# fumiama/Retrieval-based-Voice-Conversion-WebUI

Measured on AMD Instinct MI355X. Metric: real-time factor (audio-sec/wall-sec), 48 kHz v2, 10 s clips, retrieval + NSF-HiFi-GAN decode, higher is better.
Workload: dtype fp16 MFMA operands + fp16 inter-stage streams (ResBlock outputs, ups output of stages 1-3), fp32 accumulate / in-block residual; fp32 MFMA prefilter + fp64 verified IVF distances; 1 GPU; BASELINE configs[1]: v2/48k, 1 x 10 s clip(s) per GPU, T=1198 frames, 599 queries/clip, IVF 10000x768 nlist=256 nprobe=1 k=8 index_rate=0.75; hipgraph=True, index_blob_bytes=32376576, launcher=single process

## Files before the change

### retrieval-based-voice-conversion-webui_amd/csrc/nsf.hip

```cpp
#include <algorithm>
#include <atomic>
#include <cmath>
#include <functional>
#include <memory>
#include <string>
#include <unordered_map>

#include "common.hpp"
#include "nsf_kernels.hpp"
#include "conv_pack.hpp"
#include "rb_stream.hpp"

namespace rvcmi {

struct Geom {
    int MI, NJ, WCO, TT;
};
static Geom conv_geom(int cout) {
    Geom g;
    g.NJ = 4;
    if (cout >= 256) { g.MI = 2; g.WCO = 4; }
    else if (cout >= 128) { g.MI = 2; g.WCO = 2; }
    else if (cout >= 64) { g.MI = 2; g.WCO = 1; }
    else { g.MI = 1; g.WCO = 1; }
// ... 1008 lines not shown
    a2.in = hbuf;
    a2.in_mode = IN_OP_RAW;
    a2.out_mode = OUT_F32;
    a2.out = dst;
    a2.res = src;
    a2.res_bstride = L * C;
    for (ConvArgs* a : {&a1, &a2}) {
        a->in_bstride = L * C;
        a->Lin = (int)L;
        a->Lq = (int)L;
        a->lens = f.lens;
        a->lmul_in = a->lmul_q = lm;
        a->out_bstride = L * C;
        a->out_C = C;
    }
}

static void rb_f32_chain(const Fwd& f, const Stage& s, long L, int lm, const float** src) {
    rvcmi_nsf* h = f.h;
    char nm[48];
    snprintf(nm, sizeof(nm), "rb_c%d", s.cout);
    for (size_t j = 0; j < s.rb.size(); ++j)
        for (size_t m = 0; m < s.rb[j].size(); ++m) {
            float* dst = ydst(h, j, m);
            ConvArgs a1, a2;
            rb_pair_args(f, L, s.cout, lm, src[j], h->H.p, dst, a1, a2);
            run_conv(h, s.rb[j][m].first, a1, f.B, nm, f.st);
            run_conv(h, s.rb[j][m].second, a2, f.B, nm, f.st);
            src[j] = dst;
        }
}

static void rb_split(const Fwd& f, const Stage& s, long L, int lm, const float** src) {
    rvcmi_nsf* h = f.h;
    char nm[48];
    snprintf(nm, sizeof(nm), "rb_split_c%d", s.cout);
    for (size_t m = 0; m < max_levels(s); ++m) {
        const ConvLayer* L1[3];
        const ConvLayer* L2[3];
        ConvArgs a1[3], a2[3];
        int nj = 0;
        for (size_t j = 0; j < s.rb.size(); ++j) {
            if (m >= s.rb[j].size()) continue;
            float* dst = ydst(h, j, m);
            void* hbuf = (char*)h->H.p + (size_t)nj * (h->H.bytes / 3);
            rb_pair_args(f, L, s.cout, lm, src[j], hbuf, dst, a1[nj], a2[nj]);
            L1[nj] = &s.rb[j][m].first;
            L2[nj] = &s.rb[j][m].second;
            src[j] = dst;
            ++nj;
        }
        run_conv_jobs(h, L1, a1, nj, f.B, nm, f.st);
        run_conv_jobs(h, L2, a2, nj, f.B, nm, f.st);
    }
}

static void rb_stream(const Fwd& f, const Stage& s, const StagePlan& p, long L, int lm, const float** src) {
    rvcmi_nsf* h = f.h;
    const int C = s.cout, nk = (int)s.rb.size();
    RbStreamDesc sd[3];
    double flops = 0, bytes = 0;
    stream_jobs(f, s, L, lm, p.x0_half, p.stage_half, sd, flops, bytes);
    char nm[48];
    snprintf(nm, sizeof(nm), "rb_stream_c%d", C);
    h->prof.launch(nm, flops, bytes, f.st, [&] {
        rb_stream_launch(f.op, C, 3, sd, nk, (int)L, f.B, L * C, rb_stream_mode(h) == 1, f.st, h->opt);
    });
    HIP_CHECK(hipGetLastError());
    for (int j = 0; j < nk; ++j) src[j] = h->Ya[j].as<float>();
}

static void rb_full(const Fwd& f, const Stage& s, const StagePlan& p, long L, int lm, const float** src) {
    rvcmi_nsf* h = f.h;
    const int C = s.cout, nk = (int)s.rb.size(), B = f.B;
    char nm[48];
    snprintf(nm, sizeof(nm), "rb_full_c%d", C);
    RbFullArgs ra;
    memset(&ra, 0, sizeof(ra));
    ra.L = (int)L;
    ra.lens = f.lens;
    ra.lmul = lm;
    ra.bstride = L * C;
    ra.dbg = dbg_flags(h);
    ra.yh = p.stage_half ? 1 : 0;
    ra.xh = p.x0_half ? 1 : 0;
    ra.pad_tap = h->opt.geti("RBF_PAD_TAP", 0) != 0 ? 1 : 0;
    const int R = p.tall32 ? RBF32T_ROWS : (p.small64 ? RBF64S_ROWS : rbf_rows(C));
    int order[RVCMI_MAX_RB];
    rb_order(s, order);
    int max_tiles = 0;
    double flops = 0, bytes = 0;
    for (int oj = 0; oj < nk; ++oj) {
        const int j = order[oj];
        RbFullJob& J = ra.job[oj];
        J.src = h->X0.as<float>();
        J.dst = h->Ya[j].as<float>();
        J.nd = (int)s.rb[j].size();
        fill_rb_job(J, s.rb[j], 0, J.nd, L, B, C, flops, bytes);
        for (int m = 0; m < J.nd; ++m)
            if (J.dil[m] * (J.k - 1) / 2 + J.dil[m] > RBF_G) RVCMI_FAIL(RVCMI_ERR_INVALID, "dilation too large for the fused resblock");
        J.HL = rbf_halo(s.rb[j]);
        J.tvalid = R - 2 * J.HL;
        if (J.tvalid < R / 4) RVCMI_FAIL(RVCMI_ERR_INVALID, "resblock halo too large for the fused kernel");
        J.ntiles = (int)((L + J.tvalid - 1) / J.tvalid);
        max_tiles = std::max(max_tiles, J.ntiles);
        bytes += (double)B * L * C * ((p.stage_half ? 2 : 4) + (p.x0_half ? 2 : 4));
        src[j] = J.dst;
    }
    const size_t nblk = (size_t)max_tiles * nk * B;
    if (ra.dbg & 32) ra.ts = stamp_buffer(h, nblk * 8 * 16, f.st);
    h->prof.launch(nm, flops, bytes, f.st, [&] {
        if (f.op == RVCMI_OPERAND_BF16) launch_rbf_t<__bf16>(C, ra, max_tiles, nk, B, f.st, p.small64, p.tall32);
        else launch_rbf_t<_Float16>(C, ra, max_tiles, nk, B, f.st, p.small64, p.tall32);
    });
    HIP_CHECK(hipGetLastError());
    if (ra.dbg & 32) {
        const int nwv = p.tall32 ? RBF32T_NWV : (p.small64 ? RBF64S_NWV : (C == 64 ? RbFullGeom<64>::NWV : RBF32_NWV));
        print_stamps(h, nm, ra, nk, max_tiles, nwv, 16, nblk, f.st);
    }
}

static void rb_pair(const Fwd& f, const Stage& s, long L, int lm, const float** src) {
    rvcmi_nsf* h = f.h;
    const int op = f.op, C = s.cout, nk = (int)s.rb.size(), B = f.B;
    const int mode = rb_stream_mode(h);
    char nm[48], nms[48];
    snprintf(nm, sizeof(nm), "rb_pair_c%d", C);
    snprintf(nms, sizeof(nms), "rb_stream1_c%d", C);
    int order[RVCMI_MAX_RB];
    rb_order(s, order);
    constexpr int NWp = 8;
    for (size_t m = 0; m < max_levels(s); ++m) {
        RbPairArgs ra;
        memset(&ra, 0, sizeof(ra));
        ra.lens = f.lens;
        ra.lmul = lm;
        ra.L = (int)L;
        ra.bstride = L * C;
        ra.dbg = dbg_flags(h);
        RbStreamDesc sd[RVCMI_MAX_RB];
        float* dsts[RVCMI_MAX_RB] = {nullptr};
        int nj = 0, max_tiles = 0, max_rows = 0;
        double flops = 0, bytes = 0;
        for (int oj = 0; oj < nk; ++oj) {
            const int j = order[oj];
            if (m >= s.rb[j].size()) continue;
            RbStreamDesc& d = sd[nj];
            memset(&d, 0, sizeof(d));
            d.src = src[j];
            d.dst = dsts[j] = ydst(h, j, m);
            d.lens = f.lens;
            d.lmul = lm;
            fill_rb_job(d, s.rb[j], (int)m, 1, L, B, C, flops, bytes);
            bytes += (double)B * L * C * 8;
            RbJob& J = ra.job[nj++];
            J.src = d.src; J.dst = d.dst; J.w1 = d.w1[0]; J.w2 = d.w2[0]; J.b1 = d.b1[0]; J.b2 = d.b2[0];
            J.ct1 = d.ct1; J.ct2 = d.ct2; J.k = d.k; J.k_p = d.k_p; J.dil = d.dil[0];
            J.tt2 = rb_rows(C) - (J.k - 1);
            J.ntiles = (int)((L + J.tt2 - 1) / J.tt2);
            max_tiles = std::max(max_tiles, J.ntiles);
            max_rows = std::max(max_rows, rb_rows(C) + (J.k_p - 1) * J.dil);
        }
        const size_t nblk = (size_t)max_tiles * nj * B;
        if (ra.dbg & 32) ra.ts = stamp_buffer(h, nblk * NWp * 8, f.st);
        bool streamed = false;
        if (mode != 0 && rb_stream_supported(op, C, 1) && rb_stream_launch(op, C, 1, sd, nj, (int)L, B, L * C, mode == 1, f.st, h->opt, true))
            h->prof.launch(nms, flops, bytes, f.st, [&] { streamed = rb_stream_launch(op, C, 1, sd, nj, (int)L, B, L * C, mode == 1, f.st, h->opt); });
        if (!streamed) h->prof.launch(nm, flops, bytes, f.st, [&] { launch_rb_pair(op, C, ra, max_tiles, nj, B, max_rows, f.st); });
        if ((ra.dbg & 32) && m == 0) print_stamps(h, nm, ra, nj, max_tiles, NWp, 8, nblk, f.st);
        for (int j = 0; j < nk; ++j)
            if (dsts[j]) src[j] = dsts[j];
    }
    HIP_CHECK(hipGetLastError());
}

static void conv_post(const Fwd& f, const Act& x, float* out) {
    rvcmi_nsf* h = f.h;
    const int B = f.B, C = x.C, L = (int)x.L;
    hipStream_t st = f.st;
    const int dbg = h->opt.geti("POST_DBG", 0);
    h->prof.launch("conv_post", 2.0 * 7 * C * (double)x.L * B, (double)B * x.L * (C * h->cfg.n_resblock_kernels * (x.half ? 2 : 4) + 4), st, [&] {
        if (x.half && x.y[1] && x.y[2] && x.div == 3.f && (C == 32 || C == 16) && h->opt.geti("POST_DMA", 1) != 0) {
            const int ntiles = (L + POSTD_TT - 1) / POSTD_TT;
            const dim3 grid((unsigned)std::min(ntiles, std::max(1, num_cus() * 3 / B)), B);
            const _Float16* y0 = (const _Float16*)x.y[0];
            const _Float16* y1 = (const _Float16*)x.y[1];
            const _Float16* y2 = (const _Float16*)x.y[2];
            if (C == 32)
                hipLaunchKernelGGL(k_post_dma<32>, grid, dim3(POSTD_TT), post_dma_smem<32>(), st, y0, y1, y2, h->post_w.as<float>(), out, L, f.lens, x.lm, dbg);
            else
                hipLaunchKernelGGL(k_post_dma<16>, grid, dim3(POSTD_TT), post_dma_smem<16>(), st, y0, y1, y2, h->post_w.as<float>(), out, L, f.lens, x.lm, dbg);
            return;
        }
        const size_t smem = (size_t)(7 * C + (POST_TT + 6) * (C + 4)) * 4;
        hipLaunchKernelGGL(k_post, dim3((unsigned)((L + POST_TT - 1) / POST_TT), B), dim3(256), smem, st, x.y[0], x.y[1], x.y[2],
                           h->post_w.as<float>(), out, L, C, x.div, x.half ? 1 : 0, f.lens, x.lm, dbg);
    });
    HIP_CHECK(hipGetLastError());
}

static void tap_x0(const Fwd& f, const StagePlan& p, long L, int C) {
    rvcmi_nsf* h = f.h;
    if (!p.x0_half) return copy_tap_cl(h, h->X0.as<float>(), f.B, (int)L, C, f.tr, f.st);
    const size_t n = (size_t)f.B * L * C;
    hipLaunchKernelGGL(k_h2f, dim3((unsigned)((n + 255) / 256)), dim3(256), 0, f.st, (const _Float16*)h->X0.p, h->Ya[0].as<float>(), n);
    copy_tap_cl(h, h->Ya[0].as<float>(), f.B, (int)L, C, f.tr, f.st);
}

static void tap_stage(const Fwd& f, const Act& x) {
    rvcmi_nsf* h = f.h;
    const size_t n = (size_t)f.B * x.L * x.C;
    const dim3 grid((unsigned)((n + 255) / 256));
    if (x.half)
        hipLaunchKernelGGL(k_sum3h, grid, dim3(256), 0, f.st, (const _Float16*)x.y[0], (const _Float16*)x.y[1], (const _Float16*)x.y[2],
                           h->X0.as<float>(), n);
    else
        hipLaunchKernelGGL(k_sum3, grid, dim3(256), 0, f.st, x.y[0], x.y[1], x.y[2], h->X0.as<float>(), n);
    copy_tap_cl(h, h->X0.as<float>(), f.B, (int)x.L, x.C, f.tr, f.st);
}

static void nsf_forward(rvcmi_nsf* h, int B, int T, const int* lens, const float* x, const float* f0, const float* g,
                        const float* noise, int n_res, float* out, hipStream_t st, TapRequest* tr) {
    if (!h || !x || (!out && !tr)) RVCMI_FAIL(RVCMI_ERR_INVALID, "null argument");
    if (lens && n_res >= 0) RVCMI_FAIL(RVCMI_ERR_INVALID, "lengths and n_res (the realtime interpolation) cannot be combined");
    const rvcmi_nsf_config& c = h->cfg;
    if (c.use_f0 && !f0) RVCMI_FAIL(RVCMI_ERR_INVALID, "f0 is required for an NSF (use_f0) generator");
    if (B < 1 || T < 1) RVCMI_FAIL(RVCMI_ERR_INVALID, "B and T must be positive");
    const int Te = n_res >= 0 ? n_res : T;
    if (Te < 1) RVCMI_FAIL(RVCMI_ERR_INVALID, "n_res must be positive");
    if (B > h->max_B || T > h->max_T || Te > h->max_T)
        RVCMI_FAIL(RVCMI_ERR_NOMEM, "shape B=%d T=%d n_res=%d exceeds handle limits (max_B=%d max_T=%d)", B, T, n_res,
                   h->max_B, h->max_T);
    HIP_CHECK(hipSetDevice(h->device));
    Fwd f{h, c.operand, B, Te, lens, nullptr, st, tr};
    if (c.use_f0 && excitation(f, T, f0, noise)) return;
    Act a = conv_pre(f, x, T, g);
    if (f.want("pre")) return copy_tap_cl(h, a.y[0], B, Te, h->C0, tr, st);
    char nm[48];
    for (int i = 0; i < c.n_ups; ++i) {
        const Stage& s = h->stages[i];
        const long L = a.L * s.u;
        const int lm = a.lm * s.u, C = s.cout;
        const StagePlan p = plan_stage(f, s, L, lm);
        if (f.op == RVCMI_OPERAND_F32) ups_f32(f, s, a, L, lm);
        else ups_mfma(f, s, a, p, L, lm);
        snprintf(nm, sizeof(nm), "up%d", i);
        if (f.want(nm)) return tap_x0(f, p, L, C);
        const float* src[RVCMI_MAX_RB];
        for (auto& v : src) v = h->X0.as<float>();
        switch (p.path) {
            case RbPath::F32_CHAIN: rb_f32_chain(f, s, L, lm, src); break;
            case RbPath::SPLIT: rb_split(f, s, L, lm, src); break;
            case RbPath::STREAM: rb_stream(f, s, p, L, lm, src); break;
            case RbPath::FULL: rb_full(f, s, p, L, lm, src); break;
            case RbPath::PAIR: rb_pair(f, s, L, lm, src); break;
        }
        const int nk = (int)s.rb.size();
        a = Act{{src[0], nk > 1 ? src[1] : nullptr, nk > 2 ? src[2] : nullptr}, p.stage_half, false, (float)nk, L, C, lm};
        snprintf(nm, sizeof(nm), "stage%d", i);
        if (f.want(nm)) return tap_stage(f, a);
    }
    if (tr) RVCMI_FAIL(RVCMI_ERR_INVALID, "unknown tap '%s'", tr->what);
    conv_post(f, a, out);
}

}

extern "C" {

int rvcmi_nsf_create(const rvcmi_nsf_config* cfg, const rvcmi_tensor* weights, int n_weights, int device, int max_B,
                     int max_T, rvcmi_nsf** out) {
    return guarded([&] { nsf_create(cfg, weights, n_weights, device, max_B, max_T, out); });
}
int rvcmi_nsf_destroy(rvcmi_nsf* h) {
    return guarded([&] { delete h; });
}
int rvcmi_nsf_forward(rvcmi_nsf* h, int B, int T, const int* lengths, const float* x, const float* f0, const float* g,
                      const float* noise, int n_res, float* out, void* stream) {
    return guarded([&] { nsf_forward(h, B, T, lengths, x, f0, g, noise, n_res, out, (hipStream_t)stream, nullptr); });
}
int rvcmi_nsf_upp(const rvcmi_nsf* h) { return h ? h->upp : RVCMI_ERR_INVALID; }
size_t rvcmi_nsf_workspace_bytes(const rvcmi_nsf* h) { return h ? h->ws_bytes : 0; }

int rvcmi_nsf_debug_forward(rvcmi_nsf* h, int B, int T, const float* x, const float* f0, const float* g,
                            const float* noise, int n_res, const char* what, float* out_host, size_t capacity_floats,
                            int64_t shape_out[3], void* stream) {
    return guarded([&] {
        if (!what || !out_host || !shape_out) RVCMI_FAIL(RVCMI_ERR_INVALID, "null argument");
        TapRequest tr;
        tr.what = what;
        tr.out_host = out_host;
        tr.capacity = capacity_floats;
        tr.shape = shape_out;
        nsf_forward(h, B, T, nullptr, x, f0, g, noise, n_res, nullptr, (hipStream_t)stream, &tr);
        if (!tr.done) RVCMI_FAIL(RVCMI_ERR_INVALID, "tap '%s' was not produced", what);
    });
}

int rvcmi_nsf_set_option(rvcmi_nsf* h, const char* key, double value) {
    return guarded([&] {
        if (!h || !key) RVCMI_FAIL(RVCMI_ERR_INVALID, "null argument");
        if ((!strcmp(key, "RBF_PAD_TAP") || !strcmp(key, "RBF32_TALL")) && value == value && value != 0.0 && value != 1.0)
            RVCMI_FAIL(RVCMI_ERR_INVALID, "option '%s' takes 0 or 1", key);
        if (!h->opt.set(key, value)) RVCMI_FAIL(RVCMI_ERR_INVALID, "unknown option '%s' for this handle", key);
    });
}
int rvcmi_nsf_profile_enable(rvcmi_nsf* h, int enable) {
    return guarded([&] {
        if (!h) RVCMI_FAIL(RVCMI_ERR_INVALID, "null handle");
        h->prof.enabled = enable != 0;
    });
}
int rvcmi_nsf_profile_read(rvcmi_nsf* h, rvcmi_kernel_stat* stats, int capacity, int* n, int reset) {
    return guarded([&] {
        if (!h) RVCMI_FAIL(RVCMI_ERR_INVALID, "null handle");
        h->prof.read(stats, capacity, n, reset);
    });
}

}
```

### retrieval-based-voice-conversion-webui_amd/csrc/nsf_kernels.hpp

```cpp
#pragma once
#include <hip/hip_runtime.h>

#include "exact_fp.hpp"
#include <stdint.h>

namespace rvcmi {

using bf16x8 = __attribute__((ext_vector_type(8))) __bf16;
using f16x8 = __attribute__((ext_vector_type(8))) _Float16;
using f32x16 = __attribute__((ext_vector_type(16))) float;
using f32x4 = __attribute__((ext_vector_type(4))) float;

__device__ __forceinline__ float lrelu(float v, float slope) { return v > 0.f ? v : v * slope; }

__device__ __forceinline__ int item_rows(const int* __restrict__ lens, int b, int mul, int Lmax) {
    return lens ? max(min(Lmax, lens[b] * mul), min(Lmax, mul)) : Lmax;
}


static __global__ void __launch_bounds__(256) k_phase_scan(const float* __restrict__ f0, float* __restrict__ phase,
                                                   int T, float sr, float upp, const int* __restrict__ lens) {
#pragma clang fp contract(off)
    __shared__ double wsum[4];
    const int b = blockIdx.x;
// ... 184 lines not shown
    const int co = (int)(i - (size_t)t * C);
    const float* h = har + (size_t)b * Lh;
    float acc = bn[co];
    const int base = t * s - pad;
    for (int j = 0; j < k; ++j) {
        int r = base + j;
        if (r >= 0 && r < Lhb) acc = fmaf(h[r], Wn[(size_t)j * C + co], acc);
    }
    x[((size_t)b * L + t) * C + co] += acc;
}

__device__ __forceinline__ _Float16 sat_h(float v) { return (_Float16)__builtin_amdgcn_fmed3f(v, -65504.f, 65504.f); }
__device__ __forceinline__ uint2 pack4_h(float a, float b, float c, float d) {
    using h4 = __attribute__((ext_vector_type(4))) _Float16;
    h4 o = {sat_h(a), sat_h(b), sat_h(c), sat_h(d)};
    return __builtin_bit_cast(uint2, o);
}
__device__ __forceinline__ void unpack8_h(const uint4 raw, float (&f)[8]) {
    using h8 = __attribute__((ext_vector_type(8))) _Float16;
    const h8 h = __builtin_bit_cast(h8, raw);
#pragma unroll
    for (int e = 0; e < 8; ++e) f[e] = (float)h[e];
}

constexpr int POST_TT = 256;
static __global__ void __launch_bounds__(256) k_post(const float* __restrict__ xa, const float* __restrict__ xb,
                                              const float* __restrict__ xc, const float* __restrict__ Wp ,
                                              float* __restrict__ out, int Lmax, int C, float div, int in_half,
                                              const int* __restrict__ lens, int lmul, int dbg = 0 ) {
    extern __shared__ __attribute__((aligned(16))) char smem_raw[];
    float* w = (float*)smem_raw;
    float* tile = w + 7 * C;
    const int b = blockIdx.y;
    const int S = C + 4;
    for (int i = threadIdx.x; i < 7 * C; i += 256) w[i] = Wp[i];
    const int C4 = C >> 2;
    const int L = item_rows(lens, b, lmul, Lmax);
    const size_t boff = (size_t)b * Lmax * C;
    const int ntiles = (Lmax + POST_TT - 1) / POST_TT;
    for (int ti = blockIdx.x; ti < ntiles; ti += gridDim.x) {
        const int t0 = ti * POST_TT;
        if (t0 >= L) {
            if (t0 + (int)threadIdx.x < Lmax) out[(size_t)b * Lmax + t0 + threadIdx.x] = 0.f;
            continue;
        }
        constexpr int SB = 5;
        const int total = (POST_TT + 6) * C4;
        if (in_half) {
            const int C8 = C >> 3;
            const int total8 = (POST_TT + 6) * C8;
            const _Float16 *ha = (const _Float16*)xa, *hb = (const _Float16*)xb, *hc = (const _Float16*)xc;
            for (int base = threadIdx.x; base < total8; base += SB * 256) {
                uint4 va[SB], vb[SB], vc[SB];
                size_t off[SB];
#pragma unroll
                for (int u = 0; u < SB; ++u) {
                    const int idx = min(base + u * 256, total8 - 1);
                    const int r = idx / C8, c8 = idx - r * C8;
                    const int tc = min(max(t0 - 3 + r, 0), L - 1);
                    off[u] = boff + (size_t)tc * C + c8 * 8;
                    va[u] = *(const uint4*)(ha + off[u]);
                }
                if (xb) {
#pragma unroll
                    for (int u = 0; u < SB; ++u) vb[u] = *(const uint4*)(hb + off[u]);
                }
                if (xc) {
#pragma unroll
                    for (int u = 0; u < SB; ++u) vc[u] = *(const uint4*)(hc + off[u]);
                }
#pragma unroll
                for (int u = 0; u < SB; ++u) {
                    const int idx = base + u * 256;
                    if (idx < total8) {
                        const int r = idx / C8, c8 = idx - r * C8;
                        const int t = t0 - 3 + r;
                        float v[8], w2[8];
                        unpack8_h(va[u], v);
                        if (xb) {
                            unpack8_h(vb[u], w2);
#pragma unroll
                            for (int e = 0; e < 8; ++e) v[e] += w2[e];
                        }
                        if (xc) {
                            unpack8_h(vc[u], w2);
#pragma unroll
                            for (int e = 0; e < 8; ++e) v[e] += w2[e];
                        }
#pragma unroll
                        for (int e = 0; e < 8; ++e) {
                            float x = v[e];
                            if (div == 3.f) x = div3_exact(x);
                            else if (div != 1.f) x = x / div;
                            x = lrelu(x, 0.01f);
                            v[e] = (t < 0 || t >= L) ? 0.f : x;
                        }
                        *(float4*)(tile + r * S + c8 * 8) = make_float4(v[0], v[1], v[2], v[3]);
                        *(float4*)(tile + r * S + c8 * 8 + 4) = make_float4(v[4], v[5], v[6], v[7]);
                    }
                }
            }
        } else
        for (int base = threadIdx.x; base < total; base += SB * 256) {
            float4 va[SB], vb[SB], vc[SB];
            size_t off[SB];
#pragma unroll
            for (int u = 0; u < SB; ++u) {
                const int idx = min(base + u * 256, total - 1);
                const int r = idx / C4, c4 = idx - r * C4;
                const int tc = min(max(t0 - 3 + r, 0), L - 1);
                off[u] = boff + (size_t)tc * C + c4 * 4;
                va[u] = *(const float4*)(xa + off[u]);
            }
            if (xb) {
#pragma unroll
                for (int u = 0; u < SB; ++u) vb[u] = *(const float4*)(xb + off[u]);
            }
            if (xc) {
#pragma unroll
                for (int u = 0; u < SB; ++u) vc[u] = *(const float4*)(xc + off[u]);
            }
#pragma unroll
            for (int u = 0; u < SB; ++u) {
                const int idx = base + u * 256;
                if (idx < total) {
                    const int r = idx / C4, c4 = idx - r * C4;
                    const int t = t0 - 3 + r;
                    float4 v = va[u];
                    if (xb) { v.x += vb[u].x; v.y += vb[u].y; v.z += vb[u].z; v.w += vb[u].w; }
                    if (xc) { v.x += vc[u].x; v.y += vc[u].y; v.z += vc[u].z; v.w += vc[u].w; }
                    if (div == 3.f) { v.x = div3_exact(v.x); v.y = div3_exact(v.y); v.z = div3_exact(v.z); v.w = div3_exact(v.w); }
                    else if (div != 1.f) { v.x = v.x / div; v.y = v.y / div; v.z = v.z / div; v.w = v.w / div; }
                    v.x = lrelu(v.x, 0.01f); v.y = lrelu(v.y, 0.01f); v.z = lrelu(v.z, 0.01f); v.w = lrelu(v.w, 0.01f);
                    if (t < 0 || t >= L) v = make_float4(0.f, 0.f, 0.f, 0.f);
                    *(float4*)(tile + r * S + c4 * 4) = v;
                }
            }
        }
        __syncthreads();
        const int t = t0 + threadIdx.x;
        if (dbg & 2) {
            if (threadIdx.x == 0) out[(size_t)b * Lmax + t0] = tile[0];
            __syncthreads();
            continue;
        }
        if (t < L) {
            float acc = 0.f;
            for (int j = 0; j < 7; ++j) {
                const float4* row = (const float4*)(tile + (threadIdx.x + j) * S);
                const float4* wj = (const float4*)(w + j * C);
                for (int c = 0; c < C4; ++c) {
                    const float4 xv = row[c], wv = wj[c];
                    acc = fmaf(xv.x, wv.x, acc);
                    acc = fmaf(xv.y, wv.y, acc);
                    acc = fmaf(xv.z, wv.z, acc);
                    acc = fmaf(xv.w, wv.w, acc);
                }
            }
            out[(size_t)b * Lmax + t] = tanhf(acc);
        } else if (t < Lmax) {
            out[(size_t)b * Lmax + t] = 0.f;
        }
        __syncthreads();
    }
}

__device__ __forceinline__ void lds_barrier();
__device__ __forceinline__ void glds16(const void* g, unsigned lds_off) {
    unsigned keep;
    asm volatile("s_mov_b32 %0, m0\n\ts_mov_b32 m0, %2\n\ts_nop 0\n\tglobal_load_lds_dwordx4 %1, off\n\ts_mov_b32 m0, %0"
                 : "=&s"(keep)
                 : "v"(g), "s"(lds_off)
                 : "memory");
}
constexpr int POSTD_TT = 128;
template <int C>
static __global__ void __launch_bounds__(POSTD_TT) k_post_dma(const _Float16* __restrict__ xa, const _Float16* __restrict__ xb,
                                                             const _Float16* __restrict__ xc, const float* __restrict__ Wp ,
                                                             float* __restrict__ out, int Lmax, const int* __restrict__ lens, int lmul,
                                                             int dbg ) {
    constexpr int TT = POSTD_TT, NW = TT / 64, S = C + 4, C8 = C / 8, ROWB = C * 2;
    constexpr int TILEB = (TT + 6) * ROWB;
    constexpr int NP = (TILEB + 1023) / 1024, RAWB = NP * 1024;
    constexpr int PPW0 = (3 * NP + NW - 1) / NW;
    extern __shared__ __attribute__((aligned(16))) char smem_raw[];
    float* w = (float*)smem_raw;
    float* tile = w + 7 * C;
    char* raw = (char*)(tile + (TT + 6) * S);
    const int b = blockIdx.y;
    const int tid = threadIdx.x, lane = tid & 63;
    const int wave = __builtin_amdgcn_readfirstlane(tid >> 6);
    for (int i = tid; i < 7 * C; i += TT) w[i] = Wp[i];
    const int L = item_rows(lens, b, lmul, Lmax);
    const size_t boff = (size_t)b * Lmax * C;
    const int nvalid = (L + TT - 1) / TT, nall = (Lmax + TT - 1) / TT;
    const char* src[3] = {(const char*)(xa + boff), (const char*)(xb + boff), (const char*)(xc + boff)};
    const unsigned raw_off = __builtin_amdgcn_readfirstlane((unsigned)(size_t)(const __attribute__((address_space(3))) char*)raw);

    auto issue = [&](int ti) {
        if (dbg & 1) return;
        const int t0 = ti * TT;
#pragma unroll
        for (int p0 = 0; p0 < PPW0; ++p0) {
            const int p = p0 * NW + wave;
            if (p < 3 * NP) {
                const int st = p / NP, pp = p - st * NP;
                const int o = pp * 1024 + lane * 16;
                const int r = o / ROWB, col = o - r * ROWB;
                const int tc = min(max(t0 - 3 + r, 0), L - 1);
                glds16(src[st] + (size_t)tc * ROWB + col, raw_off + (unsigned)(st * RAWB + pp * 1024));
            }
        }
    };

    int ti = blockIdx.x;
    if (ti < nvalid) issue(ti);
    for (; ti < nvalid; ti += gridDim.x) {
        const int t0 = ti * TT;
        asm volatile("s_waitcnt vmcnt(0)" ::: "memory");
        lds_barrier();
        if (dbg & 2) {
            lds_barrier();
            if (ti + (int)gridDim.x < nvalid) issue(ti + gridDim.x);
            if (tid == 0) out[(size_t)b * Lmax + t0] = *(const float*)raw;
            continue;
        }
        for (int idx = tid; idx < (TT + 6) * C8; idx += TT) {
            const int r = idx / C8, c8 = idx - r * C8;
            const int t = t0 - 3 + r;
            float v[8], u[8];
            unpack8_h(*(const uint4*)(raw + r * ROWB + c8 * 16), v);
            unpack8_h(*(const uint4*)(raw + RAWB + r * ROWB + c8 * 16), u);
#pragma unroll
            for (int e = 0; e < 8; ++e) v[e] += u[e];
            unpack8_h(*(const uint4*)(raw + 2 * RAWB + r * ROWB + c8 * 16), u);
            const bool in = t >= 0 && t < L;
#pragma unroll
            for (int e = 0; e < 8; ++e) v[e] = in ? lrelu(div3_exact(v[e] + u[e]), 0.01f) : 0.f;
            *(float4*)(tile + r * S + c8 * 8) = make_float4(v[0], v[1], v[2], v[3]);
            *(float4*)(tile + r * S + c8 * 8 + 4) = make_float4(v[4], v[5], v[6], v[7]);
        }
        lds_barrier();
        if (ti + (int)gridDim.x < nvalid) issue(ti + gridDim.x);
        const int t = t0 + tid;
        float acc = 0.f;
#pragma unroll
        for (int j = 0; j < 7; ++j) {
            const float4* row = (const float4*)(tile + (tid + j) * S);
            const float4* wj = (const float4*)(w + j * C);
#pragma unroll
            for (int c = 0; c < C / 4; ++c) {
                const float4 xv = row[c], wv = wj[c];
                acc = fmaf(xv.x, wv.x, acc);
                acc = fmaf(xv.y, wv.y, acc);
                acc = fmaf(xv.z, wv.z, acc);
                acc = fmaf(xv.w, wv.w, acc);
            }
        }
        if (t < L) out[(size_t)b * Lmax + t] = tanhf(acc);
        else if (t < Lmax) out[(size_t)b * Lmax + t] = 0.f;
    }
    asm volatile("s_waitcnt vmcnt(0)" ::: "memory");
    for (ti = blockIdx.x; ti < nall; ti += gridDim.x)
        if (ti >= nvalid && ti * TT + tid < Lmax) out[(size_t)b * Lmax + ti * TT + tid] = 0.f;
}
template <int C>
static constexpr size_t post_dma_smem() {
    return (size_t)(7 * C + (POSTD_TT + 6) * (C + 4)) * 4 + (size_t)3 * (((POSTD_TT + 6) * C * 2 + 1023) / 1024) * 1024;
}

static __global__ void __launch_bounds__(256) k_sum3h(const _Float16* __restrict__ a, const _Float16* __restrict__ b,
                                               const _Float16* __restrict__ c, float* __restrict__ y, size_t n) {
    size_t i = (size_t)blockIdx.x * 256 + threadIdx.x;
    if (i < n) y[i] = ((float)a[i] + (b ? (float)b[i] : 0.f)) + (c ? (float)c[i] : 0.f);
}
static __global__ void __launch_bounds__(256) k_h2f(const _Float16* __restrict__ a, float* __restrict__ y, size_t n) {
    size_t i = (size_t)blockIdx.x * 256 + threadIdx.x;
    if (i < n) y[i] = (float)a[i];
}
static __global__ void __launch_bounds__(256) k_sum3(const float* __restrict__ a, const float* __restrict__ b,
                                              const float* __restrict__ c, float* __restrict__ y, size_t n) {
    size_t i = (size_t)blockIdx.x * 256 + threadIdx.x;
    if (i < n) y[i] = (a[i] + (b ? b[i] : 0.f)) + (c ? c[i] : 0.f);
}

static __global__ void __launch_bounds__(256) k_cl_to_cf(const float* __restrict__ in, float* __restrict__ out, int L, int C) {
    const int b = blockIdx.y;
    const size_t i = (size_t)blockIdx.x * 256 + threadIdx.x;
    if (i >= (size_t)L * C) return;
    const int c = (int)(i / L);
    const int t = (int)(i - (size_t)c * L);
    out[(size_t)b * L * C + i] = in[((size_t)b * L + t) * C + c];
}


template <typename OpT>
struct Op;
template <>
struct Op<__bf16> {
    using frag = bf16x8;
    static __device__ __forceinline__ f32x16 mfma(frag a, frag b, f32x16 c) {
        return __builtin_amdgcn_mfma_f32_32x32x16_bf16(a, b, c, 0, 0, 0);
    }
};
template <>
struct Op<_Float16> {
    using frag = f16x8;
    static __device__ __forceinline__ f32x16 mfma(frag a, frag b, f32x16 c) {
        return __builtin_amdgcn_mfma_f32_32x32x16_f16(a, b, c, 0, 0, 0);
    }
};

constexpr int KGROUP = 4;

template <typename OpT>
__device__ __forceinline__ OpT to_op(float v) {
    return (OpT)v;
}
template <>
__device__ __forceinline__ _Float16 to_op<_Float16>(float v) {
    return (_Float16)__builtin_amdgcn_fmed3f(v, -65504.f, 65504.f);
}

template <int CIN>
struct Tile {
    static constexpr int CC = CIN / 16;
    static constexpr int STRIDE = CIN * 2 + 16;
    static constexpr int TAPS_PER_GROUP = (CC >= KGROUP) ? 1 : KGROUP / CC;
    static_assert(CIN % 16 == 0, "C_in must be a multiple of 16");
    static_assert((CC >= KGROUP) ? (CC % KGROUP == 0) : (KGROUP % CC == 0), "k-group must tile a tap");
};

template <typename OpT, int CIN>
__device__ __forceinline__ void stage_tile(char* smem, const ConvArgs& a, int b, int g0, int rows) {
    using frag = typename Op<OpT>::frag;
    constexpr int STRIDE = Tile<CIN>::STRIDE;
    constexpr int C8 = CIN / 8;
    const int tid = threadIdx.x;
    const int Linb = item_rows(a.lens, b, a.lmul_in, a.Lin);
    if (a.in_mode == IN_F32_CF) {
        constexpr int SBC = 4;
        const float* ip = (const float*)a.in + (size_t)b * a.in_bstride;
        const int total = rows * C8;
        for (int base = tid; base < total; base += SBC * 256) {
            float f[SBC][8];
#pragma unroll
            for (int u = 0; u < SBC; ++u) {
                const int idx = min(base + u * 256, total - 1);
                const int c8 = idx / rows, r = idx - c8 * rows;
                const int grc = min(max(g0 + r, 0), Linb - 1);
#pragma unroll
                for (int e = 0; e < 8; ++e) f[u][e] = ip[(size_t)(c8 * 8 + e) * a.cf_stride + grc];
            }
#pragma unroll
            for (int u = 0; u < SBC; ++u) {
                const int idx = base + u * 256;
                if (idx < total) {
                    const int c8 = idx / rows, r = idx - c8 * rows;
                    const int gr = g0 + r;
                    const bool ok = gr >= 0 && gr < Linb;
                    frag v;
#pragma unroll
                    for (int e = 0; e < 8; ++e) v[e] = ok ? to_op<OpT>(f[u][e]) : (OpT)0.f;
                    *(frag*)(smem + (size_t)r * STRIDE + c8 * 16) = v;
                }
            }
        }
        return;
    }
    if (a.in_mode == IN_OP_RAW || (a.in_mode == IN_F32_ACT && !a.in_b && !a.in_c && a.div_in == 1.f)) {
        constexpr int SB = 8;
        const int total = rows * C8;
        const bool raw = a.in_mode == IN_OP_RAW;
        for (int base = tid; base < total; base += SB * 256) {
            frag vr[SB];
            float4 lo[SB], hi[SB];
#pragma unroll
            for (int u = 0; u < SB; ++u) {
                const int idx = min(base + u * 256, total - 1);
                const int r = idx / C8, c8 = idx - r * C8;
                const int grc = min(max(g0 + r, 0), Linb - 1);
                if (raw) {
                    vr[u] = *(const frag*)((const OpT*)a.in + (size_t)b * a.in_bstride + (size_t)grc * CIN + c8 * 8);
                } else {
                    const float4* p = (const float4*)((const float*)a.in + (size_t)b * a.in_bstride + (size_t)grc * CIN + c8 * 8);
                    lo[u] = p[0];
                    hi[u] = p[1];
                }
            }
#pragma unroll
            for (int u = 0; u < SB; ++u) {
                const int idx = base + u * 256;
                if (idx < total) {
                    const int r = idx / C8, c8 = idx - r * C8;
                    const int gr = g0 + r;
                    const bool ok = gr >= 0 && gr < Linb;
                    frag v;
                    if (raw) {
                        v = vr[u];
                    } else {
                        const float f[8] = {lo[u].x, lo[u].y, lo[u].z, lo[u].w, hi[u].x, hi[u].y, hi[u].z, hi[u].w};
#pragma unroll
                        for (int e = 0; e < 8; ++e) v[e] = to_op<OpT>(lrelu(f[e], a.slope_in));
                    }
                    if (!ok) {
#pragma unroll
                        for (int e = 0; e < 8; ++e) v[e] = (OpT)0.f;
                    }
                    *(frag*)(smem + (size_t)r * STRIDE + c8 * 16) = v;
                }
            }
        }
        return;
    }
    for (int idx = tid; idx < rows * C8; idx += 256) {
        const int r = idx / C8;
        const int c8 = idx - r * C8;
        const int gr = g0 + r;
        frag v;
#pragma unroll
        for (int e = 0; e < 8; ++e) v[e] = (OpT)0.f;
        if (a.in_mode == IN_HAR) {
            const long base = (long)gr * a.hs - a.hpad + c8 * 8;
            if (c8 * 8 < a.hs) {
                const float* hp = (const float*)a.in + (size_t)b * a.in_bstride;
                const float4 z4 = make_float4(0.f, 0.f, 0.f, 0.f);
                const float4 lo = (base >= 0 && base + 4 <= Linb) ? *(const float4*)(hp + base) : z4;
                const float4 hi = (base + 4 >= 0 && base + 8 <= Linb) ? *(const float4*)(hp + base + 4) : z4;
                const float f[8] = {lo.x, lo.y, lo.z, lo.w, hi.x, hi.y, hi.z, hi.w};
#pragma unroll
                for (int e = 0; e < 8; ++e) v[e] = to_op<OpT>(f[e]);
            }
        } else if (gr >= 0 && gr < Linb) {
            if (a.in_mode == IN_OP_RAW) {
                v = *(const frag*)((const OpT*)a.in + (size_t)b * a.in_bstride + (size_t)gr * CIN + c8 * 8);
            } else if (a.in_mode == IN_F32_ACT) {
                const float4* p = (const float4*)((const float*)a.in + (size_t)b * a.in_bstride + (size_t)gr * CIN + c8 * 8);
                float4 lo = p[0], hi = p[1];
                float f[8] = {lo.x, lo.y, lo.z, lo.w, hi.x, hi.y, hi.z, hi.w};
                if (a.in_b) {
                    const float4* pb = (const float4*)(a.in_b + (size_t)b * a.in_bstride + (size_t)gr * CIN + c8 * 8);
                    float4 l2 = pb[0], h2 = pb[1];
                    f[0] += l2.x; f[1] += l2.y; f[2] += l2.z; f[3] += l2.w; f[4] += h2.x; f[5] += h2.y; f[6] += h2.z; f[7] += h2.w;
                }
                if (a.in_c) {
                    const float4* pc = (const float4*)(a.in_c + (size_t)b * a.in_bstride + (size_t)gr * CIN + c8 * 8);
                    float4 l2 = pc[0], h2 = pc[1];
                    f[0] += l2.x; f[1] += l2.y; f[2] += l2.z; f[3] += l2.w; f[4] += h2.x; f[5] += h2.y; f[6] += h2.z; f[7] += h2.w;
                }
#pragma unroll
                for (int e = 0; e < 8; ++e) {
                    float x = f[e];
                    if (a.div_in == 3.f) x = div3_exact(x);
                    else if (a.div_in != 1.f) x = x / a.div_in;
                    v[e] = to_op<OpT>(lrelu(x, a.slope_in));
                }
            } else {
                const float* p = (const float*)a.in + (size_t)b * a.in_bstride + (size_t)(c8 * 8) * a.cf_stride + gr;
#pragma unroll
                for (int e = 0; e < 8; ++e) v[e] = to_op<OpT>(p[(size_t)e * a.cf_stride]);
            }
        }
        *(frag*)(smem + (size_t)r * STRIDE + c8 * 16) = v;
    }
}

template <typename OpT, int MI, int KGROUP, int NB>
__device__ __forceinline__ void conv_load_group(typename Op<OpT>::frag (&Ab)[KGROUP][MI], const OpT* wlane, long ct_stride, int grp) {
    using frag = typename Op<OpT>::frag;
#pragma unroll
    for (int g = 0; g < KGROUP; ++g)
#pragma unroll
        for (int mi = 0; mi < MI; ++mi)
            Ab[g][mi] = *(const frag*)(wlane + (size_t)mi * ct_stride + (size_t)(grp * KGROUP + g) * 512);
}

template <typename OpT, int CIN, int MI, int KGROUP, int NB>
__device__ __forceinline__ void conv_prefetch(typename Op<OpT>::frag (&A)[NB][KGROUP][MI], const OpT* wlane, long ct_stride,
                                              int ntaps_p) {
    const int NG = ntaps_p * Tile<CIN>::CC / KGROUP;
#pragma unroll
    for (int i = 0; i < NB - 1; ++i)
        if (i < NG) conv_load_group<OpT, MI, KGROUP, NB>(A[i], wlane, ct_stride, i);
}

template <typename OpT, int CIN, int MI, int NJ, int KGROUP, int NB, bool REAL = false, int JT0 = 0>
__device__ __forceinline__ void conv_run(f32x16 (&acc)[MI][NJ], typename Op<OpT>::frag (&A)[NB][KGROUP][MI],
                                         const char* lds_lane, const OpT* wlane, long ct_stride, int ntaps_p, int roff,
                                         int dstep, int dbg = 0, int nks = 0) {
    using frag = typename Op<OpT>::frag;
    using TL = Tile<CIN>;
    constexpr int CC = TL::CC;
    constexpr int STRIDE = TL::STRIDE;
    static_assert((CC >= KGROUP) ? (CC % KGROUP == 0) : (KGROUP % CC == 0), "k-group must tile a tap");
    static_assert(NB >= 2 && NB <= 4, "2..4 weight buffers");
    static_assert(KGROUP % 2 == 0, "the B ping-pong needs an even k-group");
    static_assert(JT0 >= 0 && JT0 < NJ, "at least one column tile runs");
    constexpr int NJA = NJ - JT0;
    constexpr int GPT = (CC >= KGROUP) ? CC / KGROUP : 1;
    constexpr int TPG = (CC >= KGROUP) ? 1 : KGROUP / CC;
    const int NG = ntaps_p * CC / KGROUP;
    const int dS = dstep * STRIDE;
    (void)dbg;
    (void)nks;

    auto koff = [&](int k) { return (CC >= KGROUP) ? k * 32 : (k / CC) * dS + (k % CC) * 32; };
    auto readB = [&](frag(&B)[NJ], const char* base, int k) {
        const char* bp = base + koff(k);
#pragma unroll
        for (int jt = JT0; jt < NJ; ++jt) B[jt] = *(const frag*)(bp + jt * 32 * STRIDE);
    };

    const char* gb = lds_lane + roff * STRIDE;
    int gi = 0;
    const OpT* an = wlane + (size_t)min(NB - 1, NG - 1) * KGROUP * 512;
    int gn = min(NB - 1, NG - 1);

    frag Bf[2][NJ];
#ifndef RVCMI_KLOOP_V1
#pragma unroll
    for (int jt = JT0; jt < NJ; ++jt) {
        Bf[0][jt] = *(const frag*)(gb + koff(0) + jt * 32 * STRIDE);
        __builtin_amdgcn_sched_barrier(0);
    }
#else
    readB(Bf[0], gb, 0);
#endif
    for (int grp = 0; grp < NG; grp += NB) {
#pragma unroll
        for (int u = 0; u < NB; ++u) {
            const int g = grp + u;
            if (g < NG) {
                const char* gbn;
                if constexpr (CC >= KGROUP) gbn = (gi + 1 == GPT) ? gb - (GPT - 1) * KGROUP * 32 + dS : gb + KGROUP * 32;
                else gbn = gb + TPG * dS;
#ifndef RVCMI_KLOOP_V1
#pragma unroll
                for (int k = 0; k < KGROUP; ++k) {
                    if constexpr (REAL && TPG > 1)
                        if (k > 0 && k % CC == 0 && g * KGROUP + k >= nks) goto done;
                    const char* nbp = (k + 1 < KGROUP) ? gb + koff(k + 1) : gbn + koff(0);
#pragma unroll
                    for (int mi = 0; mi < MI; ++mi)
#pragma unroll
                        for (int jt = JT0; jt < NJ; ++jt) {
                            constexpr int NS = MI * NJA;
                            const int i = mi * NJA + jt - JT0;
                            acc[mi][jt] = Op<OpT>::mfma(A[u][k][mi], Bf[k & 1][jt], acc[mi][jt]);
#ifdef RVCMI_KLOOP_ABLATE
                            if (!(RVCMI_KLOOP_ABLATE & 2))
#endif
                            if (i < NJA) Bf[(k + 1) & 1][JT0 + i] = *(const frag*)(nbp + (JT0 + i) * 32 * STRIDE);
#ifdef RVCMI_KLOOP_ABLATE
                            if (!(RVCMI_KLOOP_ABLATE & 1))
#endif
                            if (i >= NS - MI)
                                A[(u + NB - 1) % NB][k][i - (NS - MI)] = *(const frag*)(an + (size_t)(i - (NS - MI)) * ct_stride + k * 512);
                            __builtin_amdgcn_sched_barrier(0);
                        }
                }
#else
#pragma unroll
                for (int k = 0; k < KGROUP; ++k) {
                    if (k + 1 < KGROUP) readB(Bf[(k + 1) & 1], gb, k + 1);
                    else readB(Bf[0], gbn, 0);
#pragma unroll
                    for (int mi = 0; mi < MI; ++mi)
                        A[(u + NB - 1) % NB][k][mi] = *(const frag*)(an + (size_t)mi * ct_stride + k * 512);
#pragma unroll
                    for (int mi = 0; mi < MI; ++mi)
#pragma unroll
                        for (int jt = JT0; jt < NJ; ++jt) acc[mi][jt] = Op<OpT>::mfma(A[u][k][mi], Bf[k & 1][jt], acc[mi][jt]);
#pragma unroll
                    for (int i = 0; i < MI * NJA; ++i) {
                        __builtin_amdgcn_sched_group_barrier(0x008, 1, 0);
                        if (i < NJA) __builtin_amdgcn_sched_group_barrier(0x100, 1, 0);
                        else if (i < NJA + MI) __builtin_amdgcn_sched_group_barrier(0x020, 1, 0);
                    }
                }
#endif
                gb = gbn;
                if constexpr (CC >= KGROUP) gi = (gi + 1 == GPT) ? 0 : gi + 1;
                if (gn < NG - 1) {
                    ++gn;
                    an += KGROUP * 512;
                }
            }
        }
    }
done:;
}

using lds_cptr_t = const __attribute__((address_space(3))) char*;
__device__ __forceinline__ unsigned lds_address(const void* p) { return (unsigned)(size_t)(lds_cptr_t)p; }
using u32x4_t = __attribute__((ext_vector_type(4))) unsigned;
__device__ __forceinline__ __amdgpu_buffer_rsrc_t weight_rsrc(const void* p) {
    return __builtin_amdgcn_make_buffer_rsrc((void*)p, 0, 0x7fffffff, 0x00020000);
}
template <typename OpT>
__device__ __forceinline__ typename Op<OpT>::frag weight_load(__amdgpu_buffer_rsrc_t r, unsigned voff, unsigned soff) {
    return __builtin_bit_cast(typename Op<OpT>::frag, __builtin_amdgcn_raw_buffer_load_b128(r, voff, soff, 0));
}
template <typename OpT, int MI>
__device__ __forceinline__ void kconv_prefetch(typename Op<OpT>::frag (&A)[8][MI], __amdgpu_buffer_rsrc_t r, unsigned loff, unsigned ctb) {
#pragma unroll
    for (int kk = 0; kk < 8; ++kk)
#pragma unroll
        for (int mi = 0; mi < MI; ++mi) A[kk][mi] = weight_load<OpT>(r, loff + kk * 1024, mi * ctb);
}
template <typename OpT, int CIN, int MI, int NJ, int STRIDE, int JT0 = 0>
__device__ __forceinline__ void kconv(f32x16 (&acc)[MI][NJ], typename Op<OpT>::frag (&A)[8][MI], unsigned lds_row, __amdgpu_buffer_rsrc_t r,
                                      unsigned loff, unsigned ctb, int ntaps, int dstep) {
    using frag = typename Op<OpT>::frag;
    constexpr int CC = CIN / 16, GPT = CC / 8;
    static_assert(CIN % 128 == 0, "kconv: C_in must be a multiple of 128");
    static_assert(JT0 >= 0 && JT0 < NJ, "kconv: at least one column tile runs");
    constexpr int NJA = NJ - JT0;
    constexpr unsigned TS = 32u * STRIDE;
    auto ld = [](unsigned a) { return *(const __attribute__((address_space(3))) frag*)(size_t)a; };
    frag Bf[2][NJ];
#pragma unroll
    for (int jt = JT0; jt < NJ; ++jt) {
        Bf[0][jt] = ld(lds_row + jt * TS);
        __builtin_amdgcn_sched_barrier(0);
    }
    const unsigned dS = (unsigned)(dstep * STRIDE);
    const int ngroups = ntaps * GPT;
    const unsigned slast = (unsigned)(ngroups - 1) * 8192u;
    unsigned soff = ngroups > 1 ? 8192u : 0u;
    int gi = 0;
    for (int g = 0; g < ngroups; ++g) {
        const unsigned nrow = (gi + 1 == GPT) ? lds_row - (unsigned)((GPT - 1) * 256) + dS : lds_row + 256u;
        unsigned b0 = lds_row, b1 = nrow;
        asm volatile("" : "+v"(b0), "+v"(b1));
#pragma unroll
        for (int kk = 0; kk < 8; ++kk) {
#pragma unroll
            for (int mi = 0; mi < MI; ++mi)
#pragma unroll
                for (int jt = JT0; jt < NJ; ++jt) {
                    constexpr int NS = MI * NJA;
                    const int i = mi * NJA + jt - JT0;
                    acc[mi][jt] = Op<OpT>::mfma(A[kk][mi], Bf[kk & 1][jt], acc[mi][jt]);
                    if (i < NJA) Bf[(kk + 1) & 1][JT0 + i] = ld((kk < 7 ? b0 + (unsigned)((kk + 1) * 32) : b1) + (JT0 + i) * TS);
                    if (i >= NS - MI) A[kk][i - (NS - MI)] = weight_load<OpT>(r, loff + kk * 1024, soff + (unsigned)(i - (NS - MI)) * ctb);
                    __builtin_amdgcn_sched_barrier(0);
                }
        }
        lds_row = nrow;
        gi = (gi + 1 == GPT) ? 0 : gi + 1;
        soff = soff < slast ? soff + 8192u : soff;
    }
}

template <typename OpT, int CIN, int MI, int NJ, int KGROUP = ::rvcmi::KGROUP, int NB = 2>
__device__ __forceinline__ void conv_core(f32x16 (&acc)[MI][NJ], const char* lds_lane, const OpT* wlane,
                                          long ct_stride, int ntaps_p, int roff, int dstep) {
    typename Op<OpT>::frag A[NB][KGROUP][MI];
    conv_prefetch<OpT, CIN, MI, KGROUP, NB>(A, wlane, ct_stride, ntaps_p);
    conv_run<OpT, CIN, MI, NJ, KGROUP, NB>(acc, A, lds_lane, wlane, ct_stride, ntaps_p, roff, dstep);
}

template <typename OpT, int CIN, int MI, int NJ, int WCO, int NB = 2, bool PFW = false>
__device__ __forceinline__ void conv_mfma_body(const ConvArgs& a, int b, char* smem) {
    using TL = Tile<CIN>;
    constexpr int WT = 4 / WCO;
    constexpr int TT = WT * NJ * 32;
    const int ph = a.nphase > 1 ? (int)(blockIdx.y % a.nphase) : 0;
    const int cob = a.nphase > 1 ? (int)(blockIdx.y / a.nphase) : (int)blockIdx.y;
    const int q0 = blockIdx.x * TT;
    const int in_off = a.nphase > 1 ? a.ph_in_off[ph] : a.in_off;
    const OpT* wbase = (const OpT*)a.w + (a.nphase > 1 ? a.ph_w_off[ph] : 0);

    unsigned pf_acc = 0;
    if constexpr (PFW) {
        const char* wb = (const char*)(wbase + (size_t)cob * WCO * MI * a.w_ct_stride);
        const size_t bytes = (size_t)WCO * MI * a.w_ct_stride * sizeof(OpT);
        const size_t rounds = bytes / 4096;
#pragma unroll 8
        for (size_t r = 0; r < rounds; ++r) {
            const uint4 v = *(const uint4*)(wb + r * 4096 + threadIdx.x * 16);
            pf_acc ^= v.x ^ v.y ^ v.z ^ v.w;
        }
    }
    stage_tile<OpT, CIN>(smem, a, b, q0 + in_off - a.roff, a.tile_rows);
    if constexpr (PFW) {
        if (pf_acc == 0x9e3779b9u && a.Lq < 0) *(unsigned*)smem = pf_acc;
    }
    __syncthreads();

    const int wave = threadIdx.x >> 6;
    const int lane = threadIdx.x & 63;
    const int wco = wave % WCO;
    const int wt = wave / WCO;
    const int ct0 = (cob * WCO + wco) * MI;
    const int tw0 = wt * NJ * 32;

    f32x16 acc[MI][NJ];
#pragma unroll
    for (int mi = 0; mi < MI; ++mi)
#pragma unroll
        for (int jt = 0; jt < NJ; ++jt)
#pragma unroll
            for (int r = 0; r < 16; ++r) acc[mi][jt][r] = 0.f;

    const char* lds_lane = smem + (size_t)(tw0 + (lane & 31)) * TL::STRIDE + (lane >> 5) * 16;
    const OpT* wlane = wbase + (size_t)ct0 * a.w_ct_stride + lane * 8;
    conv_core<OpT, CIN, MI, NJ, KGROUP, NB>(acc, lds_lane, wlane, a.w_ct_stride, a.ntaps, a.roff, a.dstep);

    const int out_add = a.nphase > 1 ? ph : a.out_add;
    f32x4 bvec[MI][4];
#pragma unroll
    for (int mi = 0; mi < MI; ++mi)
#pragma unroll
        for (int g = 0; g < 4; ++g) bvec[mi][g] = f32x4{0.f, 0.f, 0.f, 0.f};
    if (a.bias) {
#pragma unroll
        for (int mi = 0; mi < MI; ++mi)
#pragma unroll
            for (int g = 0; g < 4; ++g) bvec[mi][g] = *(const f32x4*)(a.bias + min((ct0 + mi) * 32 + 4 * (lane >> 5) + 8 * g, a.cout - 4));
    }
    if (a.cb) {
#pragma unroll
        for (int mi = 0; mi < MI; ++mi)
#pragma unroll
            for (int g = 0; g < 4; ++g)
                bvec[mi][g] += *(const f32x4*)(a.cb + (size_t)b * a.cout + min((ct0 + mi) * 32 + 4 * (lane >> 5) + 8 * g, a.cout - 4));
    }
#pragma unroll
    for (int mi = 0; mi < MI; ++mi) {
        const int cobase = (ct0 + mi) * 32 + 4 * (lane >> 5);
#pragma unroll
        for (int jt = 0; jt < NJ; ++jt) {
            const int q = q0 + tw0 + jt * 32 + (lane & 31);
            if (q >= item_rows(a.lens, b, a.lmul_q, a.Lq)) continue;
            const size_t orow = (size_t)q * a.out_mul + out_add;
#pragma unroll
            for (int g = 0; g < 4; ++g) {
                const int co = cobase + 8 * g;
                if (co >= a.cout) continue;
                f32x4 v = {acc[mi][jt][4 * g + 0], acc[mi][jt][4 * g + 1], acc[mi][jt][4 * g + 2], acc[mi][jt][4 * g + 3]};
                v += bvec[mi][g];
                if (a.out_mode == OUT_ACT) {
                    using o4 = __attribute__((ext_vector_type(4))) OpT;
                    o4 o;
#pragma unroll
                    for (int e = 0; e < 4; ++e) o[e] = to_op<OpT>(lrelu(v[e], a.slope_out));
                    *(o4*)((OpT*)a.out + (size_t)b * a.out_bstride + orow * a.out_C + co) = o;
                } else {
                    if (a.res) v += *(const f32x4*)(a.res + (size_t)b * a.res_bstride + orow * a.out_C + co);
                    f32x4* o = (f32x4*)((float*)a.out + (size_t)b * a.out_bstride + orow * a.out_C + co);
                    if (a.accumulate) v += *o;
                    *o = v;
                }
            }
        }
    }
}

template <typename OpT, int CIN, int MI, int NJ, int WCO>
static __global__ void __launch_bounds__(256) k_conv_mfma(ConvArgs a) {
    extern __shared__ __attribute__((aligned(16))) char smem[];
    conv_mfma_body<OpT, CIN, MI, NJ, WCO>(a, (int)blockIdx.z, smem);
}

struct ConvJobs {
    ConvArgs job[3];
    int njobs;
};
template <typename OpT, int CIN, int MI, int NJ>
__device__ __forceinline__ void conv_ks_body(const ConvArgs& a, int b, char* smem) {
    using TL = Tile<CIN>;
    constexpr int CC = TL::CC;
    constexpr int TT = 32 * NJ;
    static_assert(CC >= KGROUP, "K split by taps: a tap must be whole k-groups");
    const int cob = (int)blockIdx.y;
    const int q0 = blockIdx.x * TT;
    const int wave = threadIdx.x >> 6, lane = threadIdx.x & 63;
    const int ct0 = cob * MI;
    const OpT* wbase = (const OpT*)a.w;
    const int per = (a.ntaps + 3) / 4;
    const int t0 = min(wave * per, a.ntaps), t1 = min(t0 + per, a.ntaps);
    unsigned pf_acc = 0;
    {
        const char* wb = (const char*)(wbase + (size_t)ct0 * a.w_ct_stride + (size_t)t0 * CC * 512);
        for (int r = 0; r < (t1 - t0) * CC; ++r)
#pragma unroll
            for (int mi = 0; mi < MI; ++mi) {
                const uint4 v = *(const uint4*)(wb + ((size_t)mi * a.w_ct_stride + (size_t)r * 512) * sizeof(OpT) + lane * 16);
                pf_acc ^= v.x ^ v.y ^ v.z ^ v.w;
            }
    }
    const int cobase = ct0 * 32 + 4 * (lane >> 5);
    const int Lqb = item_rows(a.lens, b, a.lmul_q, a.Lq);
    f32x4 bvec[MI][4], rvec[MI][NJ][4];
    if (wave == 0) {
#pragma unroll
        for (int mi = 0; mi < MI; ++mi)
#pragma unroll
            for (int g = 0; g < 4; ++g) {
                const int co = min(cobase + mi * 32 + 8 * g, a.cout - 4);
                bvec[mi][g] = a.bias ? *(const f32x4*)(a.bias + co) : f32x4{0.f, 0.f, 0.f, 0.f};
                if (a.cb) bvec[mi][g] += *(const f32x4*)(a.cb + (size_t)b * a.cout + co);
#pragma unroll
                for (int jt = 0; jt < NJ; ++jt) {
                    const size_t orow = (size_t)min(q0 + jt * 32 + (lane & 31), Lqb - 1) * a.out_mul + a.out_add;
                    rvec[mi][jt][g] = (a.res && a.out_mode != OUT_ACT) ? *(const f32x4*)(a.res + (size_t)b * a.res_bstride + orow * a.out_C + co)
                                                                      : f32x4{0.f, 0.f, 0.f, 0.f};
                }
            }
    }
    stage_tile<OpT, CIN>(smem, a, b, q0 + a.in_off - a.roff, a.tile_rows);
    if (pf_acc == 0x9e3779b9u && a.Lq < 0) *(unsigned*)smem = pf_acc;
    __syncthreads();

    f32x16 acc[MI][NJ];
#pragma unroll
    for (int mi = 0; mi < MI; ++mi)
#pragma unroll
        for (int jt = 0; jt < NJ; ++jt)
#pragma unroll
            for (int r = 0; r < 16; ++r) acc[mi][jt][r] = 0.f;
    const char* lds_lane = smem + (size_t)(lane & 31) * TL::STRIDE + (lane >> 5) * 16;
    if (t1 > t0)
        conv_core<OpT, CIN, MI, NJ, KGROUP, 4>(acc, lds_lane, wbase + (size_t)ct0 * a.w_ct_stride + (size_t)t0 * CC * 512 + lane * 8, a.w_ct_stride,
                                               t1 - t0, a.roff + t0 * a.dstep, a.dstep);
    float* red = (float*)(smem + (size_t)a.tile_rows * TL::STRIDE);
    if (wave > 0) {
#pragma unroll
        for (int mi = 0; mi < MI; ++mi)
#pragma unroll
            for (int jt = 0; jt < NJ; ++jt)
#pragma unroll
                for (int r = 0; r < 16; ++r) red[((((wave - 1) * MI + mi) * NJ + jt) * 16 + r) * 64 + lane] = acc[mi][jt][r];
    }
    __syncthreads();
    if (wave != 0) return;
#pragma unroll
    for (int jt = 0; jt < NJ; ++jt) {
        const int q = q0 + jt * 32 + (lane & 31);
        if (q >= Lqb) continue;
        const size_t orow = (size_t)q * a.out_mul + a.out_add;
#pragma unroll
        for (int mi = 0; mi < MI; ++mi)
#pragma unroll
            for (int g = 0; g < 4; ++g) {
                const int co = cobase + mi * 32 + 8 * g;
                if (co >= a.cout) continue;
                f32x4 v;
#pragma unroll
                for (int e = 0; e < 4; ++e) {
                    const int r = 4 * g + e;
                    v[e] = ((acc[mi][jt][r] + red[(((0 * MI + mi) * NJ + jt) * 16 + r) * 64 + lane]) + red[(((1 * MI + mi) * NJ + jt) * 16 + r) * 64 + lane]) +
                           red[(((2 * MI + mi) * NJ + jt) * 16 + r) * 64 + lane];
                }
                v += bvec[mi][g];
                if (a.out_mode == OUT_ACT) {
                    using o4 = __attribute__((ext_vector_type(4))) OpT;
                    o4 o;
#pragma unroll
                    for (int e = 0; e < 4; ++e) o[e] = to_op<OpT>(lrelu(v[e], a.slope_out));
                    *(o4*)((OpT*)a.out + (size_t)b * a.out_bstride + orow * a.out_C + co) = o;
                } else {
                    if (a.res) v += rvec[mi][jt][g];
                    f32x4* o = (f32x4*)((float*)a.out + (size_t)b * a.out_bstride + orow * a.out_C + co);
                    if (a.accumulate) v += *o;
                    *o = v;
                }
            }
    }
}
template <typename OpT, int CIN, int MI, int NJ>
static __global__ void __launch_bounds__(256) k_conv_ks_jobs(ConvJobs js) {
    extern __shared__ __attribute__((aligned(16))) char smem[];
    const int j = (int)blockIdx.z % js.njobs, b = (int)blockIdx.z / js.njobs;
    conv_ks_body<OpT, CIN, MI, NJ>(js.job[j], b, smem);
}

__device__ __forceinline__ float lrelu_max(float v, float slope) { return __builtin_amdgcn_fmed3f(v, v * slope, __builtin_inff()); }
__device__ __forceinline__ float mask_bits(float v, unsigned m) { return __uint_as_float(__float_as_uint(v) & m); }

template <typename OpT>
__device__ __forceinline__ float lrelu_op(float v) {
    return __builtin_amdgcn_fmed3f(v, v * 0.1f, 3.4028235e38f);
}
template <>
__device__ __forceinline__ float lrelu_op<_Float16>(float v) {
    return __builtin_amdgcn_fmed3f(v, v * 0.1f, 65504.f);
}
template <typename OpT, bool MASK>
__device__ __forceinline__ uint2 pack4_lrelu(float a, float b, float c, float d, unsigned m) {
    using o4 = __attribute__((ext_vector_type(4))) OpT;
    o4 o = {(OpT)lrelu_op<OpT>(a), (OpT)lrelu_op<OpT>(b), (OpT)lrelu_op<OpT>(c), (OpT)lrelu_op<OpT>(d)};
    uint2 u = __builtin_bit_cast(uint2, o);
    if constexpr (MASK) {
        u.x &= m;
        u.y &= m;
    }
    return u;
}

template <typename OpT, int C, int MI, int NJ, int STRIDE, bool MASK>
__device__ __forceinline__ void publish_operand(char* base, const f32x16 (&acc)[MI][NJ], const unsigned (&rowmask)[NJ],
                                                int cbase = 0) {
#pragma unroll
    for (int mi = 0; mi < MI; ++mi)
#pragma unroll
        for (int jt = 0; jt < NJ; ++jt)
#pragma unroll
            for (int g = 0; g < 4; ++g) {
                if ((C % 32 == 0) || cbase + mi * 32 + 8 * g < C) {
                    const f32x16& t = acc[mi][jt];
                    *(uint2*)(base + jt * 32 * STRIDE + (mi * 32 + 8 * g) * 2) =
                        pack4_lrelu<OpT, MASK>(t[4 * g + 0], t[4 * g + 1], t[4 * g + 2], t[4 * g + 3], rowmask[jt]);
                }
            }
}

__device__ __forceinline__ void lds_barrier() {
    __builtin_amdgcn_fence(__ATOMIC_RELEASE, "workgroup", "local");
    __builtin_amdgcn_s_barrier();
    __builtin_amdgcn_fence(__ATOMIC_ACQUIRE, "workgroup", "local");
}



struct RbJob {
    const float* src;
    float* dst;
    const void* w1;
    const void* w2;
    const float* b1;
    const float* b2;
    long ct1, ct2;
    int k_p;
    int k;
    int dil;
    int tt2;
    int ntiles;
};
struct RbPairArgs {
    RbJob job[4];
    int L;
    const int* lens;
    int lmul;
    long bstride;
    int dbg;
    unsigned long long* ts;
};

constexpr int RB_ROWS = 128;

template <typename OpT, int C, int MI, int NW, int KG, int NJ_ = RB_ROWS / 32, int NWT = 1, int OCC = 2>
static __global__ void __launch_bounds__(64 * NW * NWT, OCC) k_rb_pair(RbPairArgs a) {
    constexpr int ROWS = 32 * NJ_ * NWT;
    using TL = Tile<C>;
    using frag = typename Op<OpT>::frag;
    constexpr int STRIDE = TL::STRIDE;
    constexpr int C8 = C / 8;
    constexpr int NT = 64 * NW * NWT;
    constexpr int NJ = NJ_;
    constexpr int NB = 2;
    constexpr int CP = 32 * MI * NW;
    extern __shared__ __attribute__((aligned(16))) char smem[];

    const int bjob = blockIdx.y, btile = blockIdx.x;
    const RbJob& J = a.job[bjob];
    if (btile >= J.ntiles) return;
    const int b = blockIdx.z;
    const int Lb = item_rows(a.lens, b, a.lmul, a.L);
    if (btile * J.tt2 >= Lb) return;
    const int p2 = (J.k - 1) / 2;
    const int p1 = J.dil * (J.k - 1) / 2;
    const int t0 = btile * J.tt2;
    const int h0 = t0 - p2;
    const int x0 = h0 - p1;
    const int xrows = ROWS + (J.k_p - 1) * J.dil;
    const float* src = J.src + (size_t)b * a.bstride;
    float* bias_l = (float*)(smem + (size_t)xrows * STRIDE);
    unsigned long long* tsl = (unsigned long long*)(bias_l + 2 * CP);
    int tsn = 0;
    auto stamp = [&]() {
#ifdef RVCMI_DEV_STAMPS
        if ((a.dbg & 32) && (threadIdx.x & 63) == 0 && tsn < 8) tsl[(threadIdx.x >> 6) * 8 + tsn] = __builtin_readcyclecounter();
#endif
        ++tsn;
    };
    stamp();

    const int wave = threadIdx.x >> 6;
    const int lane = threadIdx.x & 63;
    const int ct0 = (wave % NW) * MI;
    const int slab = (wave / NW) * 32 * NJ_;
    const int half4 = 4 * (lane >> 5);

    frag A[NB][KG][MI];
    conv_prefetch<OpT, C, MI, KG, NB>(A, (const OpT*)J.w1 + (size_t)ct0 * J.ct1 + lane * 8, J.ct1, J.k_p);

#ifndef RB_SB
#define RB_SB 12
#endif
    constexpr int SB = RB_SB;
    const int total = xrows * C8;
    for (int base = threadIdx.x; base < total; base += SB * NT) {
        float4 lo[SB], hi[SB];
#pragma unroll
        for (int u = 0; u < SB; ++u) {
            const int idx = min(base + u * NT, total - 1);
            const int r = idx / C8;
            const int c8 = idx - r * C8;
            const int gr = x0 + r;
            const int grc = min(max(gr, 0), Lb - 1);
            const float4* p = (const float4*)(src + (size_t)grc * C + c8 * 8);
            lo[u] = p[0];
            hi[u] = p[1];
            if (gr < 0 || gr >= Lb) {
                lo[u] = make_float4(0.f, 0.f, 0.f, 0.f);
                hi[u] = lo[u];
            }
        }
#pragma unroll
        for (int u = 0; u < SB; ++u) {
            const int idx = base + u * NT;
            if (idx >= total) continue;
            const int r = idx / C8;
            const int c8 = idx - r * C8;
            const float f[8] = {lo[u].x, lo[u].y, lo[u].z, lo[u].w, hi[u].x, hi[u].y, hi[u].z, hi[u].w};
            frag v;
#pragma unroll
            for (int e = 0; e < 8; ++e) v[e] = (OpT)lrelu_op<OpT>(f[e]);
            *(frag*)(smem + (size_t)r * STRIDE + c8 * 16) = v;
        }
    }
    for (int i = threadIdx.x; i < 2 * CP; i += NT) {
        const int c = i % CP;
        bias_l[i] = c < C ? (i < CP ? J.b1[c] : J.b2[c]) : 0.f;
    }
    stamp();
    __syncthreads();
    stamp();

    const char* lds_lane = smem + (size_t)(slab + (lane & 31)) * STRIDE + (lane >> 5) * 16;
    f32x16 acc[MI][NJ];
    auto init_bias = [&](const float* bl) {
#pragma unroll
        for (int mi = 0; mi < MI; ++mi)
#pragma unroll
            for (int g = 0; g < 4; ++g) {
                const f32x4 bv = *(const f32x4*)(bl + (ct0 + mi) * 32 + 8 * g + half4);
#pragma unroll
                for (int jt = 0; jt < NJ; ++jt)
#pragma unroll
                    for (int e = 0; e < 4; ++e) acc[mi][jt][4 * g + e] = bv[e];
            }
    };

    init_bias(bias_l);
    if (!(a.dbg & 2))
        conv_run<OpT, C, MI, NJ, KG, NB>(acc, A, lds_lane, (const OpT*)J.w1 + (size_t)ct0 * J.ct1 + lane * 8, J.ct1, J.k_p, 0, J.dil);
    conv_prefetch<OpT, C, MI, KG, NB>(A, (const OpT*)J.w2 + (size_t)ct0 * J.ct2 + lane * 8, J.ct2, J.k_p);
    stamp();
    __syncthreads();

    {
        const bool interior = h0 >= 0 && h0 + ROWS <= Lb;
        unsigned rowmask[NJ];
#pragma unroll
        for (int jt = 0; jt < NJ; ++jt) {
            const int th = h0 + slab + jt * 32 + (lane & 31);
            rowmask[jt] = (th >= 0 && th < Lb) ? 0xffffffffu : 0u;
        }
        char* hw = smem + (size_t)(slab + (lane & 31)) * STRIDE + (ct0 * 32 + half4) * 2;
        if (interior) publish_operand<OpT, C, MI, NJ, STRIDE, false>(hw, acc, rowmask, ct0 * 32);
        else publish_operand<OpT, C, MI, NJ, STRIDE, true>(hw, acc, rowmask, ct0 * 32);
    }
    stamp();
    __syncthreads();
    stamp();

    init_bias(bias_l + CP);
    if (!(a.dbg & 4))
        conv_run<OpT, C, MI, NJ, KG, NB>(acc, A, lds_lane, (const OpT*)J.w2 + (size_t)ct0 * J.ct2 + lane * 8, J.ct2, J.k_p, 0, 1);

    stamp();
    float* dst = J.dst + (size_t)b * a.bstride;
#pragma unroll
    for (int jt = 0; jt < NJ; ++jt) {
        const int o = slab + jt * 32 + (lane & 31);
        const int t = t0 + o;
        const bool valid = o < J.tt2 && t < Lb;
        const int tc = min(t, Lb - 1);
        f32x4 r[MI][4];
#pragma unroll
        for (int mi = 0; mi < MI; ++mi)
#pragma unroll
            for (int g = 0; g < 4; ++g)
                if ((ct0 + mi) * 0 + mi * 32 + 8 * g < CP)
                    r[mi][g] = (C % 32 == 0 || (ct0 + mi) * 32 + 8 * g + half4 < C)
                                   ? *(const f32x4*)(src + (size_t)tc * C + min((ct0 + mi) * 32 + 8 * g + half4, C - 4))
                                   : f32x4{0.f, 0.f, 0.f, 0.f};
        if (valid && !(a.dbg & 16)) {
#pragma unroll
            for (int mi = 0; mi < MI; ++mi)
#pragma unroll
                for (int g = 0; g < 4; ++g) {
                    const int co = (ct0 + mi) * 32 + 8 * g + half4;
                    if ((C % 32 != 0) && co >= C) continue;
                    f32x4 v = {acc[mi][jt][4 * g + 0], acc[mi][jt][4 * g + 1], acc[mi][jt][4 * g + 2], acc[mi][jt][4 * g + 3]};
                    v += r[mi][g];
                    *(f32x4*)(dst + (size_t)t * C + co) = v;
                }
        }
    }
    stamp();
#ifdef RVCMI_DEV_STAMPS
    if ((a.dbg & 32) && (threadIdx.x & 63) < 8) {
        const size_t blk = ((size_t)blockIdx.z * gridDim.y + blockIdx.y) * gridDim.x + blockIdx.x;
        a.ts[(blk * NW * NWT + (threadIdx.x >> 6)) * 8 + (threadIdx.x & 63)] = tsl[(threadIdx.x >> 6) * 8 + (threadIdx.x & 63)];
    }
#endif
}

struct UpsArgs {
    const float* in_a;
    const float* in_b;
    const float* in_c;
    int in_half;
    int in_raw;
    float div;
    int Lin, cin;
    long in_bstride;
    const void* w;
    long ct_stride;
    long ph_w_off[16];
    int ph_in_off[16];
    int ntaps_p, u, cout;
    int lo;
    int tile_rows;
    const float* bias;
    float* out;
    int out_half;
    int out_tr;
    int out_tr_off;
    int out_tw_off;
    long out_bstride;
    const float* addend;
    const float* har;
    int Lh;
    int Lh_stride;
    const int* lens;
    int lmul, lhmul;
    const float* Wn;
    const float* bn;
    int nk, ns, npad;
    const void* wnz;
    int nz_k1;
    int nvt, cog, vpw;
    int dbg;
    int bias_off;
};

template <typename OpT, int CIN, int MI, int WV, int NJ = 4>
#ifndef UPS_OCC
#define UPS_OCC 2
#endif
static __global__ void __launch_bounds__(256, UPS_OCC) k_ups(UpsArgs a) {
    using TL = Tile<CIN>;
    using frag = typename Op<OpT>::frag;
    constexpr int STRIDE = TL::STRIDE;
    constexpr int C8 = CIN / 8;
    constexpr int WT = 4 / WV;
    constexpr int TQ = 32 * NJ * WT;
    constexpr int SB = 5;
    extern __shared__ __attribute__((aligned(16))) char smem[];
    const int b = blockIdx.z;
    const int q0 = blockIdx.x * TQ;
    const int Linb = item_rows(a.lens, b, a.lmul, a.Lin), Lhb = item_rows(a.lens, b, a.lhmul, a.Lh);
    if (q0 >= Linb) return;
    const int g0 = q0 + a.lo;
    const size_t boff = (size_t)b * a.in_bstride;

    const int us = a.u * a.ns;
    const long hbase = (long)q0 * us - a.npad;
    const int hspan = TQ * us + 16;
    float hpre[2] = {0.f, 0.f};
    if (a.nz_k1) {
        const float* hp = a.har + (size_t)b * a.Lh_stride;
#pragma unroll
        for (int j = 0; j < 2; ++j) {
            const long idx = hbase + (int)threadIdx.x + 256 * j;
            const long idc = min(max(idx, 0L), (long)Lhb - 1);
            const float v = hp[idc];
            hpre[j] = (idx >= 0 && idx < Lhb && (int)threadIdx.x + 256 * j < hspan) ? v : 0.f;
        }
    }
    float* bias_l = (float*)(smem + a.bias_off);
    if (a.bias_off) {
        for (int i = threadIdx.x; i < 2 * a.cout; i += 256) bias_l[i] = i < a.cout ? a.bias[i] : (a.bn ? a.bn[i - a.cout] : 0.f);
    }
    const int total = a.tile_rows * C8;
    auto convert_store = [&](int idx, float (&f)[8], bool ok) {
        const int r = idx / C8;
        const int c8 = idx - r * C8;
        if (!ok) {
#pragma unroll
            for (int e = 0; e < 8; ++e) f[e] = 0.f;
        }
        frag v;
        if (a.div == 3.f) {
#pragma unroll
            for (int e = 0; e < 8; ++e) v[e] = (OpT)lrelu_op<OpT>(div3_exact(f[e]));
        } else {
#pragma unroll
            for (int e = 0; e < 8; ++e) {
                float x = f[e];
                if (a.div != 1.f) x = x / a.div;
                v[e] = to_op<OpT>(lrelu(x, 0.1f));
            }
        }
// ... 610 lines not shown
```

### retrieval-based-voice-conversion-webui_amd/csrc/rb_stream.hip

```cpp
#include <algorithm>
#include <atomic>
#include <cmath>
#include <array>
#include <cstdlib>
#include <mutex>
#include <utility>
#include <vector>

#include "common.hpp"
#include "rb_stream.hpp"
#include "rb_stream_kernels.hpp"

namespace rvcmi {
namespace {

#ifndef RS_KL_DEFAULT
#define RS_KL_DEFAULT 2
#endif

struct Geo {
    int MI, NJ, NCO, bpc;
    double c0;
};
bool geo_for(int C, int nd, Geo& g, const Options& opt) {
    const bool sm = opt.geti("RS_SMALL", 1) != 0;
    if (C == 256 && nd == 1) { g = {2, sm ? 3 : 4, 4, 1, 4.4}; return true; }
    if (C == 128 && nd == 3) { g = {1, sm ? 6 : 8, 4, 1, opt.get("RS_C0", (sm && opt.geti("RS_KL", RS_KL_DEFAULT) == 2) ? 3.8 : 4.4)}; return true; }
    return false;
}


template <typename OpT, int C, int MI, int NJ, int NCO, int ND, int KG = 4, int NB = 2, int OCC = 1, int KL = 1, int XH = 0>
void launch_inst(const RbStreamArgs& a, int nblocks, int B, size_t smem, hipStream_t st) {
    static std::atomic<unsigned long long> attr_done{0};
    int dev = 0;
    HIP_CHECK(hipGetDevice(&dev));
    const unsigned long long bit = 1ull << (dev & 63);
    auto kern = &k_rb_stream<OpT, C, MI, NJ, NCO, ND, KG, NB, OCC, KL, XH>;
    if (!(attr_done.load() & bit)) {
        HIP_CHECK(hipFuncSetAttribute(reinterpret_cast<const void*>(kern), hipFuncAttributeMaxDynamicSharedMemorySize, 160 * 1024));
        attr_done.fetch_or(bit);
    }
    if (nblocks < 0) return;
    hipLaunchKernelGGL(kern, dim3((unsigned)nblocks * (unsigned)B), dim3(64 * NCO), smem, st, a);
}


#ifndef RS_KG128
#define RS_KG128 4
#endif
#ifndef RS_NB128
#define RS_NB128 2
#endif
template <typename OpT>
void launch_t(int C, int nd, int NJ, const RbStreamArgs& a, int nblocks, int B, size_t smem, hipStream_t st) {
    if (C == 256 && nd == 1 && NJ == 4) return launch_inst<OpT, 256, 2, 4, 4, 1>(a, nblocks, B, smem, st);
    if (C == 256 && nd == 1 && NJ == 3) return launch_inst<OpT, 256, 2, 3, 4, 1>(a, nblocks, B, smem, st);
    if (C == 128 && nd == 3 && NJ == 8) return launch_inst<OpT, 128, 1, 8, 4, 3>(a, nblocks, B, smem, st);
    if (C == 128 && nd == 3 && NJ == 6 && (a.flags & 4) && (a.flags & 16))
        return launch_inst<OpT, 128, 1, 6, 4, 3, RS_KG128, RS_NB128, 1, 2, 1>(a, nblocks, B, smem, st);
    if (C == 128 && nd == 3 && NJ == 6 && (a.flags & 4)) return launch_inst<OpT, 128, 1, 6, 4, 3, RS_KG128, RS_NB128, 1, 2>(a, nblocks, B, smem, st);
    if (C == 128 && nd == 3 && NJ == 6) return launch_inst<OpT, 128, 1, 6, 4, 3, RS_KG128, RS_NB128>(a, nblocks, B, smem, st);
    RVCMI_FAIL(RVCMI_ERR_INVALID, "rb_stream: no instantiation for C=%d nd=%d", C, nd);
}

}

void rb_stream_prepare() {
    RbStreamArgs a;
    memset(&a, 0, sizeof(a));
    for (int nj : {4, 3}) {
        launch_t<__bf16>(256, 1, nj, a, -1, 1, 0, nullptr);
        launch_t<_Float16>(256, 1, nj, a, -1, 1, 0, nullptr);
    }
    for (int nj : {8, 6}) {
        launch_t<__bf16>(128, 3, nj, a, -1, 1, 0, nullptr);
        launch_t<_Float16>(128, 3, nj, a, -1, 1, 0, nullptr);
    }
    for (int fl : {4, 4 | 16}) {
        a.flags = fl;
        launch_t<__bf16>(128, 3, 6, a, -1, 1, 0, nullptr);
        launch_t<_Float16>(128, 3, 6, a, -1, 1, 0, nullptr);
    }
    a.flags = 0;
}

bool rb_stream_supported(int operand, int C, int nd) {
    Geo g;
    return operand != RVCMI_OPERAND_F32 && geo_for(C, nd, g, Options());
}

static bool launch_geo(const Geo& g, int min_steps_required, int operand, int C, int nd, const RbStreamDesc* jobs, int njobs, int L, int B,
                       long bstride, hipStream_t st, const Options& opt, bool dry_run);

bool rb_stream_launch(int operand, int C, int nd, const RbStreamDesc* jobs, int njobs, int L, int B, long bstride, bool force,
                      hipStream_t st, const Options& opt, bool dry_run) {
    Geo g;
    if (operand == RVCMI_OPERAND_F32 || njobs < 1 || njobs > 3) return false;
    if (!geo_for(C, nd, g, opt)) return false;
    return launch_geo(g, force ? 0 : (C == 128 ? 4 : 8), operand, C, nd, jobs, njobs, L, B, bstride, st, opt, dry_run);
}

static bool launch_geo(const Geo& g, int min_steps_required, int operand, int C, int nd, const RbStreamDesc* jobs, int njobs, int L, int B,
                       long bstride, hipStream_t st, const Options& opt, bool dry_run) {
    const int R = 32 * g.NJ;
    RbStreamArgs a;
    memset(&a, 0, sizeof(a));
    a.njobs = njobs;
    a.B = B;
    a.L = L;
    a.bstride = bstride;
    const int slots1 = std::max(njobs, num_cus() * g.bpc / std::max(1, B));
    int nblocks = 0, side_rows = 0, min_steps = 1 << 30;
    int warm[3] = {0, 0, 0};
    bool fill = nd > 1 && opt.geti("RS_FILL", 1) != 0;
    for (int j = 0; j < njobs; ++j) {
        const RbStreamDesc& d = jobs[j];
        RbStreamJob& J = a.job[j];
        J.src = d.src;
        J.dst = d.dst;
        J.ct1 = d.ct1;
        J.ct2 = d.ct2;
        J.k = d.k;
        J.k_p = d.k_p;
        const int p2 = (d.k - 1) / 2;
        int sx = 0;
        warm[j] = 32 * nd + nd * p2;
        for (int m = 0; m < nd; ++m) {
            J.w1[m] = d.w1[m];
            J.w2[m] = d.w2[m];
            J.b1[m] = d.b1[m];
            J.b2[m] = d.b2[m];
            J.dil[m] = d.dil[m];
            const int p1 = d.dil[m] * (d.k - 1) / 2;
            if (p1 + p2 > 32 || 2 * p2 > RS_HROW || p1 + p2 + d.dil[m] - 32 > RS_SLACK || 32 + p1 - p2 > RS_HEAD - RS_HROW)
                return false;
            warm[j] += p1;
            J.sx_off[m] = sx;
            sx += 32 + p1 - p2;
        }
        for (int m = 0; m < nd; ++m) {
            J.sh_off[m] = sx;
            sx += 2 * p2;
        }
        for (int m = 0; m < nd; ++m)
            for (int c = 0; c < 2; ++c) {
                const int inst = rs_fill_inst(m, g.NJ);
                if (inst > rs_fill_tile(d.k, d.dil, nd, m, c) || inst > g.NJ - 2) fill = false;
            }
        side_rows = std::max(side_rows, sx);
    }
    int nst[3] = {1, 1, 1};
    {
        struct Key { int C, nd, L, slots, R, k[3], n, c0_milli; };
        static std::mutex mu;
        static std::vector<std::pair<Key, std::array<int, 3>>> cache;
        Key key{C, nd, L, slots1, R, {jobs[0].k, njobs > 1 ? jobs[1].k : 0, njobs > 2 ? jobs[2].k : 0}, njobs, (int)std::lround(g.c0 * 1000.0)};
        bool hit = false;
        {
            std::lock_guard<std::mutex> lk(mu);
            for (auto& e : cache)
                if (!memcmp(&e.first, &key, sizeof(Key))) { nst[0] = e.second[0]; nst[1] = e.second[1]; nst[2] = e.second[2]; hit = true; break; }
        }
        if (!hit) {
            const int maxn = std::max(1, L / R);
            auto tcost = [&](int j, int n) {
                const int rows = (L + n - 1) / n;
                const int steps = (rows + warm[j] + R - 1) / R;
                return steps * (jobs[j].k + g.c0);
            };
            double best_total = 1e300;
            for (int mult = 1; mult <= (slots1 >= 64 ? 1 : 4); ++mult) {
                const int slots = slots1 * mult;
                int cand[3] = {1, 1, 1};
                double best = 1e300;
                const int lim0 = std::min(maxn, slots - (njobs - 1));
                for (int n0 = 1; n0 <= lim0; ++n0) {
                    if (njobs == 1) {
                        const double t = tcost(0, n0);
                        if (t < best) { best = t; cand[0] = n0; }
                        continue;
                    }
                    const int lim1 = std::min(maxn, slots - n0 - (njobs - 2));
                    for (int n1 = 1; n1 <= lim1; ++n1) {
                        double t = std::max(tcost(0, n0), tcost(1, n1));
                        if (t >= best) continue;
                        if (njobs == 2) { best = t; cand[0] = n0; cand[1] = n1; continue; }
                        const int n2 = std::min(maxn, slots - n0 - n1);
                        if (n2 < 1) continue;
                        t = std::max(t, tcost(2, n2));
                        if (t < best) { best = t; cand[0] = n0; cand[1] = n1; cand[2] = n2; }
                    }
                }
                if (best * mult < best_total * 0.97) {
                    best_total = best * mult;
                    nst[0] = cand[0]; nst[1] = cand[1]; nst[2] = cand[2];
                }
            }
            std::lock_guard<std::mutex> lk(mu);
            if (cache.size() > 64) cache.clear();
            cache.push_back({key, {nst[0], nst[1], nst[2]}});
        }
    }
    for (int j = 0; j < njobs; ++j) {
        RbStreamJob& J = a.job[j];
        const int rows = (L + nst[j] - 1) / nst[j];
        const int steps = (rows + warm[j] + R - 1) / R;
        const int len = std::max(rows, steps * R - warm[j]);
        J.strip_len = len;
        J.nstrips = (L + len - 1) / len;
        J.blk0 = nblocks;
        nblocks += J.nstrips;
        min_steps = std::min(min_steps, steps);
    }
    a.side_rows = side_rows;
    if (opt.geti("RS_KL", RS_KL_DEFAULT) == 2 && (double)L * C * 4.0 < 2147483648.0) a.flags = 4;
    a.lens = jobs[0].lens;
    a.lmul = jobs[0].lmul;
    if (jobs[0].y_half) a.flags |= 8;
    if (fill) a.flags |= 32;
    if (jobs[0].x_half) {
        if (!(a.flags & 4) || !(C == 128 && nd == 3 && g.NJ == 6)) return false;
        a.flags |= 16;
    }
    if (min_steps < min_steps_required) return false;
    const size_t smem = (size_t)(RS_HEAD + R + RS_SLACK + side_rows + 1) * (2 * C + 16) + (size_t)nd * 2 * C * sizeof(float);
    const bool kl2 = C == 128 && nd == 3 && g.NJ == 6 && (a.flags & 4);
    const size_t smem_kl2 = (size_t)(side_rows + 1) * (2 * C + 16) + (size_t)nd * 2 * C * sizeof(float) +
                            std::max((size_t)(RS_HEAD + R + RS_SLACK) * (2 * C + 16), (size_t)R * (4 * C + 16));
    if (kl2 && smem_kl2 > (size_t)160 * 1024) RVCMI_FAIL(RVCMI_ERR_INVALID, "rb_stream: LDS image %zu B too large (C=%d)", smem_kl2, C);
    if (smem > (size_t)160 * 1024 / g.bpc)
        RVCMI_FAIL(RVCMI_ERR_INVALID, "rb_stream: LDS image %zu B too large for %d block(s) per CU (C=%d)", smem, g.bpc, C);
    if (dry_run) return true;
    const bool want_stamps = opt.on("RS_STAMPS");
    unsigned long long* ts = nullptr;
    const size_t nts = (size_t)nblocks * B * g.NCO * 16;
    if (want_stamps) {
        HIP_CHECK(hipMalloc(&ts, nts * 8));
        HIP_CHECK(hipMemsetAsync(ts, 0, nts * 8, st));
        a.ts = ts;
    }
    if (operand == RVCMI_OPERAND_BF16) launch_t<__bf16>(C, nd, g.NJ, a, nblocks, B, kl2 ? smem_kl2 : smem, st);
    else launch_t<_Float16>(C, nd, g.NJ, a, nblocks, B, kl2 ? smem_kl2 : smem, st);
    if (want_stamps) {
        HIP_CHECK(hipStreamSynchronize(st));
        std::vector<unsigned long long> h(nts);
        HIP_CHECK(hipMemcpy(h.data(), ts, nts * 8, hipMemcpyDeviceToHost));
        (void)hipFree(ts);
        static const char* names[10] = {"phaseA", "barA", "conv1", "bar1", "phaseB", "barB", "conv2", "bar2", "xload", "store"};
        for (int j = 0; j < njobs; ++j) {
            double sum[10] = {0}, steps = 0, tot_max = 0;
            long cnt = 0;
            for (size_t w = 0; w < (size_t)nblocks * B * g.NCO; ++w) {
                const unsigned long long* p = &h[w * 16];
                if ((int)p[11] != j || !p[10]) continue;
                double tot = 0;
                for (int i = 0; i < 10; ++i) { sum[i] += (double)p[i]; tot += (double)p[i]; }
                tot_max = std::max(tot_max, tot);
                steps += (double)p[10];
                ++cnt;
            }
            if (!cnt) continue;
            fprintf(stderr, "[rs stamps] C=%d nd=%d NJ=%d k=%d strips=%d len=%d steps/blk=%.1f  cycles per PAIR-step:", C, nd, g.NJ, a.job[j].k,
                    a.job[j].nstrips, a.job[j].strip_len, steps / cnt);
            for (int i = 0; i < 8; ++i) fprintf(stderr, " %s %.0f", names[i], sum[i] / (steps * nd));
            fprintf(stderr, " | per step: xload %.0f store %.0f | slowest wave total %.0f cycles\n", sum[8] / steps, sum[9] / steps, tot_max);
        }
    }
    return true;
}

}
```

### retrieval-based-voice-conversion-webui_amd/csrc/rb_stream.hpp

```cpp
#pragma once
#include <hip/hip_runtime.h>

#include "common.hpp"

namespace rvcmi {

struct RbStreamDesc {
    const float* src;
    float* dst;
    const void* w1[3];
    const void* w2[3];
    const float* b1[3];
    const float* b2[3];
    long ct1, ct2;
    int k, k_p;
    int dil[3];
    int y_half;
    int x_half;
    const int* lens;
    int lmul;
};

void rb_stream_prepare();
bool rb_stream_supported(int operand, int C, int nd);
inline void rb_stream_load_env(Options& opt) { opt.load_env({"RS_SMALL", "RS_KL", "RS_C0", "RS_STAMPS", "RS_FILL"}); }
bool rb_stream_launch(int operand, int C, int nd, const RbStreamDesc* jobs, int njobs, int L, int B, long bstride, bool force,
                      hipStream_t st, const Options& opt, bool dry_run = false);

}
```

### retrieval-based-voice-conversion-webui_amd/csrc/rb_stream_kernels.hpp

```cpp
#pragma once
#include <type_traits>

#include "nsf_kernels.hpp"

namespace rvcmi {

constexpr int RS_HEAD = 62;
constexpr int RS_HROW = 10;
constexpr int RS_SLACK = 4;
constexpr int RS_MAXND = 3;

inline int rs_fill_tile(int k, const int* dil, int nd, int m, int conv2) {
    const int p2 = (k - 1) / 2;
    int HL = nd * p2, later = 0;
    for (int i = 0; i < nd; ++i) HL += dil[i] * (k - 1) / 2;
    for (int i = m + 1; i < nd; ++i) later += dil[i] * (k - 1) / 2 + p2;
    const int S0 = 0, r0 = S0 - HL;
    const int need = S0 - later - (conv2 ? 0 : p2);
    const int win = r0 - 32 * (m + 1) + (conv2 ? 0 : p2);
    return (need - win) / 32;
}
constexpr int rs_fill_inst(int m, int NJ) { return m + 1 <= NJ - 2 ? m + 1 : 0; }

struct RbStreamJob {
    const float* src;
    float* dst;
    const void* w1[RS_MAXND];
    const void* w2[RS_MAXND];
    const float* b1[RS_MAXND];
    const float* b2[RS_MAXND];
    long ct1, ct2;
    int k, k_p;
    int dil[RS_MAXND];
    int blk0;
    int nstrips;
    int strip_len;
    int sx_off[RS_MAXND];
    int sh_off[RS_MAXND];
};
struct RbStreamArgs {
    RbStreamJob job[3];
    int njobs;
    int B;
    int L;
    const int* lens;
    int lmul;
    long bstride;
    int side_rows;
    int flags;
    unsigned long long* ts;
};

template <int STRIDE, int NT>
__device__ __forceinline__ void rs_copy_rows(char* dst, const char* src, int rows) {
    constexpr int W = STRIDE / 16;
    const int total = rows * W;
    for (int i = threadIdx.x; i < total; i += NT) *(uint4*)(dst + (size_t)i * 16) = *(const uint4*)(src + (size_t)i * 16);
}

template <typename OpT, int C, int MI, int NJ, int NCO, int ND, int KG, int NB, int OCC = 1, int KL = 1, int XH = 0>
static __global__ void __launch_bounds__(64 * NCO, OCC) k_rb_stream(RbStreamArgs a) {
    using TL = Tile<C>;
    using frag = typename Op<OpT>::frag;
    using o4 = __attribute__((ext_vector_type(4))) OpT;
    constexpr int STRIDE = TL::STRIDE;
    constexpr int NT = 64 * NCO;
    constexpr int R = 32 * NJ;
    constexpr int CP = 32 * MI * NCO;
    static_assert(CP == C, "waves must tile the channels exactly");
    constexpr int MROWS = RS_HEAD + R + RS_SLACK;
    extern __shared__ __attribute__((aligned(16))) char smem[];
    char* side = KL == 2 ? smem : smem + (size_t)MROWS * STRIDE;
    char* dump = side + (size_t)a.side_rows * STRIDE;
    float* bias_l = (float*)(dump + STRIDE);
    char* M = KL == 2 ? (char*)(bias_l + ND * 2 * CP) : smem;

    int lb;
    {
        const int nb = (int)gridDim.x, q = nb >> 3, r = nb & 7, xcd = (int)blockIdx.x & 7, slot = (int)blockIdx.x >> 3;
        lb = (xcd < r ? xcd * (q + 1) : r * (q + 1) + (xcd - r) * q) + slot;
    }
    int ji = 0;
#pragma unroll
    for (int j = 1; j < 3; ++j)
        if (j < a.njobs && lb >= a.job[j].blk0 * a.B) ji = j;
    const RbStreamJob& J = a.job[ji];
    const int rem = lb - J.blk0 * a.B;
    const int b = rem / J.nstrips;
    const int strip = rem - b * J.nstrips;
    if (b >= a.B) return;
    const float* src = J.src + (size_t)b * a.bstride;
    float* dst = J.dst + (size_t)b * a.bstride;
    const int L = item_rows(a.lens, b, a.lmul, a.L);
    const int S0 = strip * J.strip_len;
    const int S1 = min(L, S0 + J.strip_len);
    if (S0 >= L) return;
    const int p2 = (J.k - 1) / 2;
    int HL = ND * p2;
#pragma unroll
    for (int m = 0; m < ND; ++m) HL += J.dil[m] * (J.k - 1) / 2;
    const int r0 = S0 - HL;
    const int nsteps = (S1 - r0 + 32 * ND + R - 1) / R;

    const int wave = __builtin_amdgcn_readfirstlane((int)(threadIdx.x >> 6)), lane = threadIdx.x & 63;
    const int ct0 = wave * MI;
    const int half4 = 4 * (lane >> 5);
    const int lrow = lane & 31;

    {
        const int total16 = (int)(((size_t)(MROWS + a.side_rows + 1) * STRIDE + (KL == 2 ? ND * 2 * CP * 4 : 0)) / 16);
        const uint4 z = make_uint4(0, 0, 0, 0);
        for (int i = threadIdx.x; i < total16; i += NT) *(uint4*)(smem + (size_t)i * 16) = z;
        if constexpr (KL == 2) __syncthreads();
        for (int i = threadIdx.x; i < ND * 2 * CP; i += NT) {
            const int m = i / (2 * CP), w = (i / CP) & 1, c = i % CP;
            bias_l[i] = (w ? J.b2[m] : J.b1[m])[c];
        }
    }

    unsigned long long tprev = 0, tsum[12] = {0, 0, 0, 0, 0, 0, 0, 0, 0, 0, 0, 0};
    const bool stamps = a.ts != nullptr;
    auto stamp = [&](int ph) {
        if (stamps) {
            const unsigned long long t = __builtin_readcyclecounter();
            tsum[ph] += t - tprev;
            tprev = t;
        }
    };
    if (stamps) tprev = __builtin_readcyclecounter();

    auto bar = [] {
        if constexpr (KL == 2) {
            __builtin_amdgcn_fence(__ATOMIC_RELEASE, "workgroup", "local");
            __builtin_amdgcn_s_barrier();
            __builtin_amdgcn_fence(__ATOMIC_ACQUIRE, "workgroup", "local");
        } else {
            __syncthreads();
        }
    };
    f32x16 carry[ND][MI];
#pragma unroll
    for (int m = 0; m < ND; ++m)
#pragma unroll
        for (int mi = 0; mi < MI; ++mi)
#pragma unroll
            for (int e = 0; e < 16; ++e) carry[m][mi][e] = 0.f;

    frag A[NB][KG][MI];
    frag A8[8][MI];
    const unsigned loff = (unsigned)lane * 16u;
    const unsigned ctb1 = (unsigned)(J.ct1 * 2), ctb2 = (unsigned)(J.ct2 * 2);
    auto prefetch = [&](const OpT* wl, long ct, unsigned ctb) {
        if constexpr (KL == 2) kconv_prefetch<OpT, MI>(A8, weight_rsrc(wl), loff, ctb);
        else conv_prefetch<OpT, C, MI, KG, NB>(A, wl + lane * 8, ct, J.k_p);
    };
    auto run = [&](auto jt0c, f32x16 (&acc)[MI][NJ], const char* lds_lane, const OpT* wl, long ct, unsigned ctb, int dstep) {
        constexpr int JT0 = decltype(jt0c)::value;
        if constexpr (KL == 2) kconv<OpT, C, MI, NJ, STRIDE, JT0>(acc, A8, lds_address(lds_lane), weight_rsrc(wl), loff, ctb, J.k, dstep);
        else conv_run<OpT, C, MI, NJ, KG, NB, false, JT0>(acc, A, lds_lane, wl + lane * 8, ct, J.k_p, 0, dstep);
    };
    prefetch((const OpT*)J.w1[0] + (size_t)ct0 * J.ct1, J.ct1, ctb1);
    __syncthreads();

    constexpr int CHR = C / 4;
    constexpr int NG8 = NT / CHR;
    constexpr int NCH = R / NG8;
    constexpr int TSTR = C * 4 + 16;
    static_assert(KL != 2 || (NT % CHR == 0 && R % NG8 == 0 && NCH % 8 == 0 && C * 4 * 8 == 4096), "IO chunk geometry");
    char* T = M;
    f32x4 xr[(KL == 2 && !XH) ? NCH : 1];
    u32x4_t xrh[(KL == 2 && XH) ? R / (NT / (CHR / 2)) : 1];
    constexpr bool xhf = XH != 0;
    static_assert(!xhf || KL == 2, "fp16 input rows come through the coalesced step IO");
    const __amdgpu_buffer_rsrc_t rs_src =
        xhf ? __builtin_amdgcn_make_buffer_rsrc((void*)((const _Float16*)J.src + (size_t)b * a.bstride), 0, (int)((size_t)L * C * 2), 0x00020000)
            : __builtin_amdgcn_make_buffer_rsrc((void*)src, 0, (int)((size_t)L * C * 4), 0x00020000);
    const bool yh = (a.flags & 8) != 0;
    _Float16* dsth = (_Float16*)J.dst + (size_t)b * a.bstride;
    const __amdgpu_buffer_rsrc_t rs_dst =
        yh ? __builtin_amdgcn_make_buffer_rsrc((void*)(dsth + (size_t)S0 * C), 0, (int)((size_t)max(S1 - S0, 0) * C * 2), 0x00020000)
           : __builtin_amdgcn_make_buffer_rsrc((void*)(dst + (size_t)S0 * C), 0, (int)((size_t)max(S1 - S0, 0) * C * 4), 0x00020000);
    constexpr int CHRH = CHR / 2, NG16 = NT / CHRH, NCHH = R / NG16, TSTRH = C * 2 + 16;
    static_assert(KL != 2 || (R % NG16 == 0 && (NCHH - 1) * C * 2 < 4096), "fp16 IO chunk geometry");
    const int g16 = (int)threadIdx.x / CHRH, cchh = (int)threadIdx.x % CHRH;
    const unsigned ioh_voff = (unsigned)(g16 * NCHH * C * 2 + cchh * 16);
    const unsigned ioh_lds = lds_address(T) + (unsigned)(g16 * NCHH * TSTRH + cchh * 16);
    const unsigned dlh_lds = lds_address(T) + (unsigned)(lrow * TSTRH + (ct0 * 32 + half4) * 2);
    const int g8 = (int)threadIdx.x / CHR, cch = (int)threadIdx.x % CHR;
    const unsigned io_voff = (unsigned)(g8 * NCH * C * 4 + cch * 16);
    const unsigned io_lds = lds_address(T) + (unsigned)(g8 * NCH * TSTR + cch * 16);
    auto issue_loads = [&](int w0) {
        if constexpr (xhf) {
            unsigned v0 = ioh_voff + (unsigned)(w0 * (C * 2));
            asm volatile("" : "+v"(v0));
#pragma unroll
            for (int it = 0; it < NCHH; ++it) xrh[it] = __builtin_amdgcn_raw_buffer_load_b128(rs_src, v0 + (unsigned)(it * (C * 2)), 0, 0);
        } else {
        unsigned v0[NCH / 8];
#pragma unroll
        for (int j = 0; j < NCH / 8; ++j) {
            v0[j] = io_voff + (unsigned)(w0 * (C * 4)) + (unsigned)(j * 4096);
            asm volatile("" : "+v"(v0[j]));
        }
#pragma unroll
        for (int it = 0; it < NCH; ++it)
            xr[it] = __builtin_bit_cast(f32x4, __builtin_amdgcn_raw_buffer_load_b128(rs_src, v0[it / 8] + (unsigned)((it % 8) * (C * 4)), 0, 0));
        }
    };
    const unsigned dl_lds = lds_address(T) + (unsigned)(lrow * TSTR + (ct0 * 32 + half4) * 4);
    using lds_f32x4 = __attribute__((address_space(3))) f32x4;
    if constexpr (KL == 2) issue_loads(r0);

    auto do_step = [&](auto fillc, const int step) {
        constexpr bool FILL = decltype(fillc)::value;
        f32x16 xin[MI][NJ];
        if constexpr (KL == 2) {
            bar();
            if constexpr (xhf) {
                using lds_u4i = __attribute__((address_space(3))) u32x4_t;
                using h4 = __attribute__((ext_vector_type(4))) _Float16;
                using lds_h4 = __attribute__((address_space(3))) h4;
                {
                    unsigned bb = ioh_lds;
                    asm volatile("" : "+v"(bb));
#pragma unroll
                    for (int it = 0; it < NCHH; ++it) *(lds_u4i*)(size_t)(bb + (unsigned)(it * TSTRH)) = xrh[it];
                }
                bar();
                {
                    unsigned b0 = dlh_lds;
                    asm volatile("" : "+v"(b0));
#pragma unroll
                    for (int jt = 0; jt < NJ; ++jt)
#pragma unroll
                        for (int mi = 0; mi < MI; ++mi)
#pragma unroll
                            for (int g = 0; g < 4; ++g) {
                                const h4 v = *(const lds_h4*)(size_t)(b0 + (unsigned)(jt * 32 * TSTRH + (mi * 32 + 8 * g) * 2));
#pragma unroll
                                for (int e = 0; e < 4; ++e) xin[mi][jt][4 * g + e] = (float)v[e];
                            }
                }
            } else {
            {
                unsigned b = io_lds;
                asm volatile("" : "+v"(b));
#pragma unroll
                for (int it = 0; it < NCH; ++it) *(lds_f32x4*)(size_t)(b + (unsigned)(it * TSTR)) = xr[it];
            }
            bar();
            {
                unsigned b0 = dl_lds, b1 = dl_lds + (unsigned)(3 * 32 * TSTR);
                asm volatile("" : "+v"(b0), "+v"(b1));
#pragma unroll
                for (int jt = 0; jt < NJ; ++jt)
#pragma unroll
                    for (int mi = 0; mi < MI; ++mi)
#pragma unroll
                        for (int g = 0; g < 4; ++g) {
                            const f32x4 v = *(const lds_f32x4*)(size_t)((jt < 3 ? b0 : b1) + (unsigned)((jt % 3) * 32 * TSTR + (mi * 32 + 8 * g) * 4));
#pragma unroll
                            for (int e = 0; e < 4; ++e) xin[mi][jt][4 * g + e] = v[e];
                        }
            }
            }
            bar();
        } else
        {
            const int w0 = r0 + step * R;
#pragma unroll
            for (int jt = 0; jt < NJ; ++jt) {
                const int tg = w0 + jt * 32 + lrow;
                const unsigned msk = (tg >= 0 && tg < L) ? 0xffffffffu : 0u;
                const int tgc = min(max(tg, 0), L - 1);
#pragma unroll
                for (int mi = 0; mi < MI; ++mi)
#pragma unroll
                    for (int g = 0; g < 4; ++g) {
                        const f32x4 v = *(const f32x4*)(src + (size_t)tgc * C + (ct0 + mi) * 32 + 8 * g + half4);
#pragma unroll
                        for (int e = 0; e < 4; ++e) xin[mi][jt][4 * g + e] = mask_bits(v[e], msk);
                    }
            }
        }
        stamp(8);
        auto pair = [&](auto mc) {
            constexpr int m = decltype(mc)::value;
            using jt0_t = std::integral_constant<int, FILL ? rs_fill_inst(m, NJ) : 0>;
            const int dil = J.dil[m];
            const int p1 = dil * (J.k - 1) / 2;
            const int Hx = 32 + p1 - p2;
            const int wm = r0 - 32 * m + step * R;
            const bool interior = wm - 32 >= 0 && wm + R <= L;
            char* sideX = side + (size_t)J.sx_off[m] * STRIDE;
            char* sideH = side + (size_t)J.sh_off[m] * STRIDE;
            const OpT* w1l = (const OpT*)J.w1[m] + (size_t)ct0 * J.ct1;
            const OpT* w2l = (const OpT*)J.w2[m] + (size_t)ct0 * J.ct2;

            constexpr int WB = 64 * MI;
            constexpr int WCH = WB / 16;
            constexpr int RPI = 64 / WCH;
            constexpr int NIT = (52 + RPI - 1) / RPI;
            uint4 hb[KL == 2 ? NIT : 1];
            if constexpr (KL == 2) {
#pragma unroll
                for (int it = 0; it < NIT; ++it) {
                    const int i = min(it * RPI + lane / WCH, Hx - 1);
                    hb[it] = *(const uint4*)(sideX + (size_t)i * STRIDE + ct0 * 64 + (lane % WCH) * 16);
                }
            } else {
                rs_copy_rows<STRIDE, NT>(M + (size_t)(RS_HEAD - Hx) * STRIDE, sideX, Hx);
            }
            rs_copy_rows<STRIDE, NT>(M + (size_t)(RS_HROW - 2 * p2) * STRIDE, sideH, 2 * p2);
            {
                unsigned rowmask[NJ];
#pragma unroll
                for (int jt = 0; jt < NJ; ++jt) {
                    const int t = wm + jt * 32 + lrow;
                    rowmask[jt] = (t >= 0 && t < L) ? 0xffffffffu : 0u;
                }
                char* xw = M + (size_t)(RS_HEAD + lrow) * STRIDE + (ct0 * 32 + half4) * 2;
                if (interior) publish_operand<OpT, C, MI, NJ, STRIDE, false>(xw, xin, rowmask);
                else publish_operand<OpT, C, MI, NJ, STRIDE, true>(xw, xin, rowmask);
                if constexpr (KL == 2) {
#pragma unroll
                    for (int it = 0; it < NIT; ++it) {
                        const int i = min(it * RPI + lane / WCH, Hx - 1);
                        *(uint4*)(M + (size_t)(RS_HEAD - Hx + i) * STRIDE + ct0 * 64 + (lane % WCH) * 16) = hb[it];
                    }
#pragma unroll
                    for (int jt = NJ - 2; jt < NJ; ++jt) {
                        const int srow = jt * 32 + lrow - (R - Hx);
                        char* tw = (srow >= 0 ? sideX + (size_t)srow * STRIDE : dump) + (ct0 * 32 + half4) * 2;
#pragma unroll
                        for (int mi = 0; mi < MI; ++mi)
#pragma unroll
                            for (int g = 0; g < 4; ++g) {
                                const f32x16& t = xin[mi][jt];
                                *(uint2*)(tw + (mi * 32 + 8 * g) * 2) =
                                    interior ? pack4_lrelu<OpT, false>(t[4 * g + 0], t[4 * g + 1], t[4 * g + 2], t[4 * g + 3], 0u)
                                             : pack4_lrelu<OpT, true>(t[4 * g + 0], t[4 * g + 1], t[4 * g + 2], t[4 * g + 3], rowmask[jt]);
                            }
                    }
                }
            }
            f32x16 res[MI][NJ];
#pragma unroll
            for (int mi = 0; mi < MI; ++mi) {
                res[mi][0] = carry[m][mi];
#pragma unroll
                for (int jt = 1; jt < NJ; ++jt) res[mi][jt] = xin[mi][jt - 1];
                carry[m][mi] = xin[mi][NJ - 1];
            }
            stamp(0);
            bar();
            stamp(1);

            f32x16 hacc[MI][NJ];
            {
                const float* bl = bias_l + (m * 2 + 0) * CP + ct0 * 32 + half4;
#pragma unroll
                for (int mi = 0; mi < MI; ++mi)
#pragma unroll
                    for (int g = 0; g < 4; ++g) {
                        const f32x4 bv = *(const f32x4*)(bl + mi * 32 + 8 * g);
#pragma unroll
                        for (int jt = 0; jt < NJ; ++jt)
#pragma unroll
                            for (int e = 0; e < 4; ++e) hacc[mi][jt][4 * g + e] = bv[e];
                    }
            }
            run(jt0_t{}, hacc, M + (size_t)(RS_HEAD - Hx + lrow) * STRIDE + (lane >> 5) * 16, w1l, J.ct1, ctb1, dil);
            prefetch(w2l, J.ct2, ctb2);
            stamp(2);
            bar();
            stamp(3);

            if constexpr (KL != 2) rs_copy_rows<STRIDE, NT>(sideX, M + (size_t)(RS_HEAD + R - Hx) * STRIDE, Hx);
            {
                const int am = wm - 32 + p2;
                unsigned rowmask[NJ];
#pragma unroll
                for (int jt = 0; jt < NJ; ++jt) {
                    const int t = am + jt * 32 + lrow;
                    rowmask[jt] = (t >= 0 && t < L) ? 0xffffffffu : 0u;
                }
                char* hw = M + (size_t)(RS_HROW + lrow) * STRIDE + (ct0 * 32 + half4) * 2;
                if (interior) publish_operand<OpT, C, MI, NJ, STRIDE, false>(hw, hacc, rowmask);
                else publish_operand<OpT, C, MI, NJ, STRIDE, true>(hw, hacc, rowmask);
                const int srow = lrow - (32 - 2 * p2);
                char* tw = (srow >= 0 ? sideH + (size_t)srow * STRIDE : dump) + (ct0 * 32 + half4) * 2;
#pragma unroll
                for (int mi = 0; mi < MI; ++mi)
#pragma unroll
                    for (int g = 0; g < 4; ++g) {
                        const f32x16& t = hacc[mi][NJ - 1];
                        *(uint2*)(tw + (mi * 32 + 8 * g) * 2) =
                            pack4_lrelu<OpT, true>(t[4 * g + 0], t[4 * g + 1], t[4 * g + 2], t[4 * g + 3], rowmask[NJ - 1]);
                    }
            }
            stamp(4);
            bar();
            stamp(5);

            {
                const float* bl = bias_l + (m * 2 + 1) * CP + ct0 * 32 + half4;
#pragma unroll
                for (int mi = 0; mi < MI; ++mi)
#pragma unroll
                    for (int g = 0; g < 4; ++g) {
                        const f32x4 bv = *(const f32x4*)(bl + mi * 32 + 8 * g);
#pragma unroll
                        for (int jt = 0; jt < NJ; ++jt)
#pragma unroll
                            for (int e = 0; e < 4; ++e) res[mi][jt][4 * g + e] += bv[e];
                    }
            }
            run(jt0_t{}, res, M + (size_t)(RS_HROW - 2 * p2 + lrow) * STRIDE + (lane >> 5) * 16, w2l, J.ct2, ctb2, 1);
            {
                const int mn = (m + 1 < ND) ? m + 1 : 0;
                prefetch((const OpT*)J.w1[mn] + (size_t)ct0 * J.ct1, J.ct1, ctb1);
            }
            stamp(6);
            bar();
            stamp(7);
#pragma unroll
            for (int mi = 0; mi < MI; ++mi)
#pragma unroll
                for (int jt = 0; jt < NJ; ++jt) xin[mi][jt] = res[mi][jt];
        };
        pair(std::integral_constant<int, 0>{});
        if constexpr (ND > 1) pair(std::integral_constant<int, 1>{});
        if constexpr (ND > 2) pair(std::integral_constant<int, 2>{});
        static_assert(ND <= 3, "pair calls above");
        if constexpr (KL == 2) {
            const int wout = r0 - 32 * ND + step * R;
            if (step + 1 < nsteps) issue_loads(r0 + (step + 1) * R);
            if (yh) {
                using u32x2_t = __attribute__((ext_vector_type(2))) unsigned;
                using lds_u2 = __attribute__((address_space(3))) u32x2_t;
                using lds_u4 = __attribute__((address_space(3))) u32x4_t;
                {
                    unsigned b0 = dlh_lds;
                    asm volatile("" : "+v"(b0));
#pragma unroll
                    for (int jt = 0; jt < NJ; ++jt)
#pragma unroll
                        for (int mi = 0; mi < MI; ++mi)
#pragma unroll
                            for (int g = 0; g < 4; ++g)
                                *(lds_u2*)(size_t)(b0 + (unsigned)(jt * 32 * TSTRH + (mi * 32 + 8 * g) * 2)) = __builtin_bit_cast(
                                    u32x2_t, pack4_h(xin[mi][jt][4 * g + 0], xin[mi][jt][4 * g + 1], xin[mi][jt][4 * g + 2], xin[mi][jt][4 * g + 3]));
                }
                bar();
                {
                    unsigned bb = ioh_lds;
                    unsigned v0 = ioh_voff + (unsigned)((wout - S0) * (C * 2));
                    asm volatile("" : "+v"(bb), "+v"(v0));
#pragma unroll
                    for (int it = 0; it < NCHH; ++it) {
                        const u32x4_t v = *(const lds_u4*)(size_t)(bb + (unsigned)(it * TSTRH));
                        __builtin_amdgcn_raw_buffer_store_b128(v, rs_dst, v0 + (unsigned)(it * (C * 2)), 0, 0);
                    }
                }
            } else {
            {
                unsigned b0 = dl_lds, b1 = dl_lds + (unsigned)(3 * 32 * TSTR);
                asm volatile("" : "+v"(b0), "+v"(b1));
#pragma unroll
                for (int jt = 0; jt < NJ; ++jt)
#pragma unroll
                    for (int mi = 0; mi < MI; ++mi)
#pragma unroll
                        for (int g = 0; g < 4; ++g) {
                            const f32x4 v = {xin[mi][jt][4 * g + 0], xin[mi][jt][4 * g + 1], xin[mi][jt][4 * g + 2], xin[mi][jt][4 * g + 3]};
                            *(lds_f32x4*)(size_t)((jt < 3 ? b0 : b1) + (unsigned)((jt % 3) * 32 * TSTR + (mi * 32 + 8 * g) * 4)) = v;
                        }
            }
            bar();
            {
                unsigned b = io_lds;
                asm volatile("" : "+v"(b));
                unsigned v0[NCH / 8];
#pragma unroll
                for (int j = 0; j < NCH / 8; ++j) {
                    v0[j] = io_voff + (unsigned)((wout - S0) * (C * 4)) + (unsigned)(j * 4096);
                    asm volatile("" : "+v"(v0[j]));
                }
#pragma unroll
                for (int it = 0; it < NCH; ++it) {
                    const f32x4 v = *(const lds_f32x4*)(size_t)(b + (unsigned)(it * TSTR));
                    __builtin_amdgcn_raw_buffer_store_b128(__builtin_bit_cast(u32x4_t, v), rs_dst, v0[it / 8] + (unsigned)((it % 8) * (C * 4)), 0, 0);
                }
            }
            }
        } else
        {
            const int wout = r0 - 32 * ND + step * R;
#pragma unroll
            for (int jt = 0; jt < NJ; ++jt) {
                const int tg = wout + jt * 32 + lrow;
                if (tg >= S0 && tg < S1) {
#pragma unroll
                    for (int mi = 0; mi < MI; ++mi)
#pragma unroll
                        for (int g = 0; g < 4; ++g) {
                            const f32x4 v = {xin[mi][jt][4 * g + 0], xin[mi][jt][4 * g + 1], xin[mi][jt][4 * g + 2], xin[mi][jt][4 * g + 3]};
                            if (yh) *(uint2*)(dsth + (size_t)tg * C + (ct0 + mi) * 32 + 8 * g + half4) = pack4_h(v[0], v[1], v[2], v[3]);
                            else *(f32x4*)(dst + (size_t)tg * C + (ct0 + mi) * 32 + 8 * g + half4) = v;
                        }
                }
            }
        }
        stamp(9);
    };
    int step0 = 0;
    if constexpr (ND > 1) {
        if (a.flags & 32) {
            do_step(std::true_type{}, 0);
            step0 = 1;
        }
    }
    for (int step = step0; step < nsteps; ++step) do_step(std::false_type{}, step);
    if (stamps && lane < 12) {
        unsigned long long v = 0;
#pragma unroll
        for (int i = 0; i < 12; ++i) v = (lane == i) ? tsum[i] : v;
        if (lane == 10) v = (unsigned long long)nsteps;
        if (lane == 11) v = (unsigned long long)ji;
        a.ts[((size_t)blockIdx.x * NCO + wave) * 16 + lane] = v;
    }
}

}
```

Before: 5762 x real-time (audio-sec/wall-sec), whole job.

## Add 16x16x32 MFMA path to C=128 ResBlock stream kernel

Adds a 16x16x32 MFMA variant of the lean K loop (kconv16) with new lane-to-row/chunk mappings, weight offsets, publish routine and carry/residual handling generalized to 16-row tiles. It becomes the default for the C=128, nd=3, NJ=6 stream kernel through a new flag bit and RS_MFMA option. The intent is to use the higher-throughput, lower-latency small MFMA shape and finer-grained interleaving of LDS and weight loads. In exchange it doubles the number of MFMA issues and LDS B-fragment loads per tile and adds register-layout complexity.

```diff
diff --git a/retrieval-based-voice-conversion-webui_amd/csrc/nsf.hip b/retrieval-based-voice-conversion-webui_amd/csrc/nsf.hip
--- a/retrieval-based-voice-conversion-webui_amd/csrc/nsf.hip
+++ b/retrieval-based-voice-conversion-webui_amd/csrc/nsf.hip
@@ -1334,6 +1334,7 @@
         if (!h || !key) RVCMI_FAIL(RVCMI_ERR_INVALID, "null argument");
         if ((!strcmp(key, "RBF_PAD_TAP") || !strcmp(key, "RBF32_TALL")) && value == value && value != 0.0 && value != 1.0)
             RVCMI_FAIL(RVCMI_ERR_INVALID, "option '%s' takes 0 or 1", key);
+        if (!strcmp(key, "RS_MFMA") && value == value && value != 16.0 && value != 32.0) RVCMI_FAIL(RVCMI_ERR_INVALID, "option 'RS_MFMA' takes 16 or 32");
         if (!h->opt.set(key, value)) RVCMI_FAIL(RVCMI_ERR_INVALID, "unknown option '%s' for this handle", key);
     });
 }
diff --git a/retrieval-based-voice-conversion-webui_amd/csrc/nsf_kernels.hpp b/retrieval-based-voice-conversion-webui_amd/csrc/nsf_kernels.hpp
--- a/retrieval-based-voice-conversion-webui_amd/csrc/nsf_kernels.hpp
+++ b/retrieval-based-voice-conversion-webui_amd/csrc/nsf_kernels.hpp
@@ -510,12 +510,18 @@
     static __device__ __forceinline__ f32x16 mfma(frag a, frag b, f32x16 c) {
         return __builtin_amdgcn_mfma_f32_32x32x16_bf16(a, b, c, 0, 0, 0);
     }
+    static __device__ __forceinline__ f32x4 mfma16(frag a, frag b, f32x4 c) {
+        return __builtin_amdgcn_mfma_f32_16x16x32_bf16(a, b, c, 0, 0, 0);
+    }
 };
 template <>
 struct Op<_Float16> {
     using frag = f16x8;
     static __device__ __forceinline__ f32x16 mfma(frag a, frag b, f32x16 c) {
         return __builtin_amdgcn_mfma_f32_32x32x16_f16(a, b, c, 0, 0, 0);
+    }
+    static __device__ __forceinline__ f32x4 mfma16(frag a, frag b, f32x4 c) {
+        return __builtin_amdgcn_mfma_f32_16x16x32_f16(a, b, c, 0, 0, 0);
     }
 };
 
@@ -852,6 +858,63 @@
                     acc[mi][jt] = Op<OpT>::mfma(A[kk][mi], Bf[kk & 1][jt], acc[mi][jt]);
                     if (i < NJA) Bf[(kk + 1) & 1][JT0 + i] = ld((kk < 7 ? b0 + (unsigned)((kk + 1) * 32) : b1) + (JT0 + i) * TS);
                     if (i >= NS - MI) A[kk][i - (NS - MI)] = weight_load<OpT>(r, loff + kk * 1024, soff + (unsigned)(i - (NS - MI)) * ctb);
+                    __builtin_amdgcn_sched_barrier(0);
+                }
+        }
+        lds_row = nrow;
+        gi = (gi + 1 == GPT) ? 0 : gi + 1;
+        soff = soff < slast ? soff + 8192u : soff;
+    }
+}
+
+__host__ __device__ constexpr int mfma16_row(int n) { return n < 4 ? 2 * n : n < 12 ? 2 * n - 7 : 2 * n - 16; }
+__host__ __device__ constexpr int mfma16_chunk(int q) { return ((q & 1) << 1) | (q >> 1); }
+__device__ __forceinline__ unsigned mfma16_loff(int lane) {
+    const int q = lane >> 4, n = lane & 15;
+    return (unsigned)(((q & 1) * 64 + (q >> 1) * 32 + n) * 16);
+}
+template <typename OpT, int MI>
+__device__ __forceinline__ void kconv16_prefetch(typename Op<OpT>::frag (&A)[8][MI], __amdgpu_buffer_rsrc_t r, unsigned loff, unsigned ctb) {
+    static_assert(MI == 1, "kconv16: one 32-channel tile per wave");
+#pragma unroll
+    for (int s = 0; s < 4; ++s)
+#pragma unroll
+        for (int h = 0; h < 2; ++h) A[2 * s + h][0] = weight_load<OpT>(r, loff + s * 2048 + h * 256, 0);
+}
+template <typename OpT, int CIN, int MI, int NJ, int STRIDE, int JT0 = 0>
+__device__ __forceinline__ void kconv16(f32x4 (&acc)[2 * MI][2 * NJ], typename Op<OpT>::frag (&A)[8][MI], unsigned lds_row,
+                                        __amdgpu_buffer_rsrc_t r, unsigned loff, unsigned ctb, int ntaps, int dstep) {
+    using frag = typename Op<OpT>::frag;
+    constexpr int CC = CIN / 16, GPT = CC / 8, NT = 2 * NJ;
+    static_assert(CIN % 128 == 0, "kconv16: C_in must be a multiple of 128");
+    static_assert(MI == 1, "kconv16: one 32-channel tile per wave");
+    static_assert(JT0 >= 0 && JT0 < NT, "kconv16: at least one column tile runs");
+    constexpr unsigned TS = 16u * STRIDE;
+    auto ld = [](unsigned a) { return *(const __attribute__((address_space(3))) frag*)(size_t)a; };
+    frag Bf[NT];
+#pragma unroll
+    for (int jt = JT0; jt < NT; ++jt) {
+        Bf[jt] = ld(lds_row + jt * TS);
+        __builtin_amdgcn_sched_barrier(0);
+    }
+    const unsigned dS = (unsigned)(dstep * STRIDE);
+    const int ngroups = ntaps * GPT;
+    const unsigned slast = (unsigned)(ngroups - 1) * 8192u;
+    unsigned soff = ngroups > 1 ? 8192u : 0u;
+    int gi = 0;
+    for (int g = 0; g < ngroups; ++g) {
+        const unsigned nrow = (gi + 1 == GPT) ? lds_row - (unsigned)((GPT - 1) * 256) + dS : lds_row + 256u;
+        unsigned b0 = lds_row, b1 = nrow;
+        asm volatile("" : "+v"(b0), "+v"(b1));
+#pragma unroll
+        for (int s = 0; s < 4; ++s) {
+#pragma unroll
+            for (int jt = JT0; jt < NT; ++jt)
+#pragma unroll
+                for (int h = 0; h < 2; ++h) {
+                    acc[h][jt] = Op<OpT>::mfma16(A[2 * s + h][0], Bf[jt], acc[h][jt]);
+                    if (h == 1) Bf[jt] = ld((s < 3 ? b0 + (unsigned)((s + 1) * 64) : b1) + jt * TS);
+                    if (jt == NT - 1) A[2 * s + h][0] = weight_load<OpT>(r, loff + s * 2048 + h * 256, soff);
                     __builtin_amdgcn_sched_barrier(0);
                 }
         }
@@ -1123,6 +1186,17 @@
                         pack4_lrelu<OpT, MASK>(t[4 * g + 0], t[4 * g + 1], t[4 * g + 2], t[4 * g + 3], rowmask[jt]);
                 }
             }
+}
+
+template <typename OpT, int MIH, int NT, int STRIDE, bool MASK>
+__device__ __forceinline__ void publish_operand16(char* base, const f32x4 (&acc)[MIH][NT], const unsigned (&rowmask)[NT]) {
+#pragma unroll
+    for (int mi = 0; mi < MIH; ++mi)
+#pragma unroll
+        for (int jt = 0; jt < NT; ++jt) {
+            const f32x4& t = acc[mi][jt];
+            *(uint2*)(base + jt * 16 * STRIDE + mi * 16 * 2) = pack4_lrelu<OpT, MASK>(t[0], t[1], t[2], t[3], rowmask[jt]);
+        }
 }
 
 __device__ __forceinline__ void lds_barrier() {
diff --git a/retrieval-based-voice-conversion-webui_amd/csrc/rb_stream.hip b/retrieval-based-voice-conversion-webui_amd/csrc/rb_stream.hip
--- a/retrieval-based-voice-conversion-webui_amd/csrc/rb_stream.hip
+++ b/retrieval-based-voice-conversion-webui_amd/csrc/rb_stream.hip
@@ -16,6 +16,10 @@
 
 #ifndef RS_KL_DEFAULT
 #define RS_KL_DEFAULT 2
+#endif
+
+#ifndef RS_MFMA_DEFAULT
+#define RS_MFMA_DEFAULT 16
 #endif
 
 struct Geo {
@@ -30,13 +34,13 @@
 }
 
 
-template <typename OpT, int C, int MI, int NJ, int NCO, int ND, int KG = 4, int NB = 2, int OCC = 1, int KL = 1, int XH = 0>
+template <typename OpT, int C, int MI, int NJ, int NCO, int ND, int KG = 4, int NB = 2, int OCC = 1, int KL = 1, int XH = 0, int SH = 32>
 void launch_inst(const RbStreamArgs& a, int nblocks, int B, size_t smem, hipStream_t st) {
     static std::atomic<unsigned long long> attr_done{0};
     int dev = 0;
     HIP_CHECK(hipGetDevice(&dev));
     const unsigned long long bit = 1ull << (dev & 63);
-    auto kern = &k_rb_stream<OpT, C, MI, NJ, NCO, ND, KG, NB, OCC, KL, XH>;
+    auto kern = &k_rb_stream<OpT, C, MI, NJ, NCO, ND, KG, NB, OCC, KL, XH, SH>;
     if (!(attr_done.load() & bit)) {
         HIP_CHECK(hipFuncSetAttribute(reinterpret_cast<const void*>(kern), hipFuncAttributeMaxDynamicSharedMemorySize, 160 * 1024));
         attr_done.fetch_or(bit);
@@ -57,6 +61,10 @@
     if (C == 256 && nd == 1 && NJ == 4) return launch_inst<OpT, 256, 2, 4, 4, 1>(a, nblocks, B, smem, st);
     if (C == 256 && nd == 1 && NJ == 3) return launch_inst<OpT, 256, 2, 3, 4, 1>(a, nblocks, B, smem, st);
     if (C == 128 && nd == 3 && NJ == 8) return launch_inst<OpT, 128, 1, 8, 4, 3>(a, nblocks, B, smem, st);
+    if (C == 128 && nd == 3 && NJ == 6 && (a.flags & 4) && (a.flags & 64)) {
+        if (a.flags & 16) return launch_inst<OpT, 128, 1, 6, 4, 3, RS_KG128, RS_NB128, 1, 2, 1, 16>(a, nblocks, B, smem, st);
+        return launch_inst<OpT, 128, 1, 6, 4, 3, RS_KG128, RS_NB128, 1, 2, 0, 16>(a, nblocks, B, smem, st);
+    }
     if (C == 128 && nd == 3 && NJ == 6 && (a.flags & 4) && (a.flags & 16))
         return launch_inst<OpT, 128, 1, 6, 4, 3, RS_KG128, RS_NB128, 1, 2, 1>(a, nblocks, B, smem, st);
     if (C == 128 && nd == 3 && NJ == 6 && (a.flags & 4)) return launch_inst<OpT, 128, 1, 6, 4, 3, RS_KG128, RS_NB128, 1, 2>(a, nblocks, B, smem, st);
@@ -77,7 +85,7 @@
         launch_t<__bf16>(128, 3, nj, a, -1, 1, 0, nullptr);
         launch_t<_Float16>(128, 3, nj, a, -1, 1, 0, nullptr);
     }
-    for (int fl : {4, 4 | 16}) {
+    for (int fl : {4, 4 | 16, 4 | 64, 4 | 16 | 64}) {
         a.flags = fl;
         launch_t<__bf16>(128, 3, 6, a, -1, 1, 0, nullptr);
         launch_t<_Float16>(128, 3, 6, a, -1, 1, 0, nullptr);
@@ -152,10 +160,11 @@
     }
     int nst[3] = {1, 1, 1};
     {
-        struct Key { int C, nd, L, slots, R, k[3], n, c0_milli; };
+        struct Key { int C, nd, L, slots, R, k[3], n, c0_milli, mfma; };
         static std::mutex mu;
         static std::vector<std::pair<Key, std::array<int, 3>>> cache;
-        Key key{C, nd, L, slots1, R, {jobs[0].k, njobs > 1 ? jobs[1].k : 0, njobs > 2 ? jobs[2].k : 0}, njobs, (int)std::lround(g.c0 * 1000.0)};
+        Key key{C, nd, L, slots1, R, {jobs[0].k, njobs > 1 ? jobs[1].k : 0, njobs > 2 ? jobs[2].k : 0}, njobs, (int)std::lround(g.c0 * 1000.0),
+                opt.geti("RS_MFMA", RS_MFMA_DEFAULT)};
         bool hit = false;
         {
             std::lock_guard<std::mutex> lk(mu);
@@ -217,6 +226,7 @@
     if (opt.geti("RS_KL", RS_KL_DEFAULT) == 2 && (double)L * C * 4.0 < 2147483648.0) a.flags = 4;
     a.lens = jobs[0].lens;
     a.lmul = jobs[0].lmul;
+    if ((a.flags & 4) && C == 128 && nd == 3 && g.NJ == 6 && opt.geti("RS_MFMA", RS_MFMA_DEFAULT) == 16) a.flags |= 64;
     if (jobs[0].y_half) a.flags |= 8;
     if (fill) a.flags |= 32;
     if (jobs[0].x_half) {
@@ -261,8 +271,8 @@
                 ++cnt;
             }
             if (!cnt) continue;
-            fprintf(stderr, "[rs stamps] C=%d nd=%d NJ=%d k=%d strips=%d len=%d steps/blk=%.1f  cycles per PAIR-step:", C, nd, g.NJ, a.job[j].k,
-                    a.job[j].nstrips, a.job[j].strip_len, steps / cnt);
+            fprintf(stderr, "[rs stamps] C=%d nd=%d NJ=%d k=%d strips=%d len=%d mfma=%d steps/blk=%.1f  cycles per PAIR-step:", C, nd, g.NJ, a.job[j].k,
+                    a.job[j].nstrips, a.job[j].strip_len, (a.flags & 64) ? 16 : 32, steps / cnt);
             for (int i = 0; i < 8; ++i) fprintf(stderr, " %s %.0f", names[i], sum[i] / (steps * nd));
             fprintf(stderr, " | per step: xload %.0f store %.0f | slowest wave total %.0f cycles\n", sum[8] / steps, sum[9] / steps, tot_max);
         }
diff --git a/retrieval-based-voice-conversion-webui_amd/csrc/rb_stream.hpp b/retrieval-based-voice-conversion-webui_amd/csrc/rb_stream.hpp
--- a/retrieval-based-voice-conversion-webui_amd/csrc/rb_stream.hpp
+++ b/retrieval-based-voice-conversion-webui_amd/csrc/rb_stream.hpp
@@ -23,7 +23,7 @@
 
 void rb_stream_prepare();
 bool rb_stream_supported(int operand, int C, int nd);
-inline void rb_stream_load_env(Options& opt) { opt.load_env({"RS_SMALL", "RS_KL", "RS_C0", "RS_STAMPS", "RS_FILL"}); }
+inline void rb_stream_load_env(Options& opt) { opt.load_env({"RS_SMALL", "RS_KL", "RS_C0", "RS_STAMPS", "RS_FILL", "RS_MFMA"}); }
 bool rb_stream_launch(int operand, int C, int nd, const RbStreamDesc* jobs, int njobs, int L, int B, long bstride, bool force,
                       hipStream_t st, const Options& opt, bool dry_run = false);
 
diff --git a/retrieval-based-voice-conversion-webui_amd/csrc/rb_stream_kernels.hpp b/retrieval-based-voice-conversion-webui_amd/csrc/rb_stream_kernels.hpp
--- a/retrieval-based-voice-conversion-webui_amd/csrc/rb_stream_kernels.hpp
+++ b/retrieval-based-voice-conversion-webui_amd/csrc/rb_stream_kernels.hpp
@@ -58,11 +58,14 @@
     for (int i = threadIdx.x; i < total; i += NT) *(uint4*)(dst + (size_t)i * 16) = *(const uint4*)(src + (size_t)i * 16);
 }
 
-template <typename OpT, int C, int MI, int NJ, int NCO, int ND, int KG, int NB, int OCC = 1, int KL = 1, int XH = 0>
+template <typename OpT, int C, int MI, int NJ, int NCO, int ND, int KG, int NB, int OCC = 1, int KL = 1, int XH = 0, int SH = 32>
 static __global__ void __launch_bounds__(64 * NCO, OCC) k_rb_stream(RbStreamArgs a) {
     using TL = Tile<C>;
     using frag = typename Op<OpT>::frag;
     using o4 = __attribute__((ext_vector_type(4))) OpT;
+    static_assert(SH == 32 || (SH == 16 && KL == 2 && MI == 1), "the 16x16x32 shape runs in the lean K loop only");
+    using acc_t = std::conditional_t<SH == 32, f32x16, f32x4>;
+    constexpr int TR = SH, CT = SH, LAG = 32 / TR, NTL = NJ * LAG, MIH = MI * LAG, NG = SH == 32 ? 4 : 1;
     constexpr int STRIDE = TL::STRIDE;
     constexpr int NT = 64 * NCO;
     constexpr int R = 32 * NJ;
@@ -104,8 +107,9 @@
 
     const int wave = __builtin_amdgcn_readfirstlane((int)(threadIdx.x >> 6)), lane = threadIdx.x & 63;
     const int ct0 = wave * MI;
-    const int half4 = 4 * (lane >> 5);
-    const int lrow = lane & 31;
+    const int half4 = SH == 32 ? 4 * (lane >> 5) : 4 * (lane >> 4);
+    const int lrow = SH == 32 ? lane & 31 : mfma16_row(lane & 15);
+    auto bchunk = [&] { return SH == 32 ? (lane >> 5) * 16 : mfma16_chunk(lane >> 4) * 16; };
 
     {
         const int total16 = (int)(((size_t)(MROWS + a.side_rows + 1) * STRIDE + (KL == 2 ? ND * 2 * CP * 4 : 0)) / 16);
@@ -138,26 +142,39 @@
             __syncthreads();
         }
     };
-    f32x16 carry[ND][MI];
+    acc_t carry[ND][MIH][LAG];
 #pragma unroll
     for (int m = 0; m < ND; ++m)
 #pragma unroll
-        for (int mi = 0; mi < MI; ++mi)
-#pragma unroll
-            for (int e = 0; e < 16; ++e) carry[m][mi][e] = 0.f;
+        for (int mi = 0; mi < MIH; ++mi)
+#pragma unroll
+            for (int j = 0; j < LAG; ++j)
+#pragma unroll
+                for (int e = 0; e < 4 * NG; ++e) carry[m][mi][j][e] = 0.f;
 
     frag A[NB][KG][MI];
     frag A8[8][MI];
-    const unsigned loff = (unsigned)lane * 16u;
+    const unsigned loff = SH == 32 ? (unsigned)lane * 16u : mfma16_loff(lane);
     const unsigned ctb1 = (unsigned)(J.ct1 * 2), ctb2 = (unsigned)(J.ct2 * 2);
     auto prefetch = [&](const OpT* wl, long ct, unsigned ctb) {
-        if constexpr (KL == 2) kconv_prefetch<OpT, MI>(A8, weight_rsrc(wl), loff, ctb);
+        if constexpr (SH == 16) kconv16_prefetch<OpT, MI>(A8, weight_rsrc(wl), loff, ctb);
+        else if constexpr (KL == 2) kconv_prefetch<OpT, MI>(A8, weight_rsrc(wl), loff, ctb);
         else conv_prefetch<OpT, C, MI, KG, NB>(A, wl + lane * 8, ct, J.k_p);
     };
-    auto run = [&](auto jt0c, f32x16 (&acc)[MI][NJ], const char* lds_lane, const OpT* wl, long ct, unsigned ctb, int dstep) {
+    auto run = [&](auto jt0c, acc_t (&acc)[MIH][NTL], const char* lds_lane, const OpT* wl, long ct, unsigned ctb, int dstep) {
         constexpr int JT0 = decltype(jt0c)::value;
-        if constexpr (KL == 2) kconv<OpT, C, MI, NJ, STRIDE, JT0>(acc, A8, lds_address(lds_lane), weight_rsrc(wl), loff, ctb, J.k, dstep);
+        if constexpr (SH == 16) kconv16<OpT, C, MI, NJ, STRIDE, JT0>(acc, A8, lds_address(lds_lane), weight_rsrc(wl), loff, ctb, J.k, dstep);
+        else if constexpr (KL == 2) kconv<OpT, C, MI, NJ, STRIDE, JT0>(acc, A8, lds_address(lds_lane), weight_rsrc(wl), loff, ctb, J.k, dstep);
         else conv_run<OpT, C, MI, NJ, KG, NB, false, JT0>(acc, A, lds_lane, wl + lane * 8, ct, J.k_p, 0, dstep);
+    };
+    auto publish = [&](char* base, const acc_t (&acc)[MIH][NTL], const unsigned (&rowmask)[NTL], bool interior) {
+        if constexpr (SH == 16) {
+            if (interior) publish_operand16<OpT, MIH, NTL, STRIDE, false>(base, acc, rowmask);
+            else publish_operand16<OpT, MIH, NTL, STRIDE, true>(base, acc, rowmask);
+        } else {
+            if (interior) publish_operand<OpT, C, MI, NJ, STRIDE, false>(base, acc, rowmask);
+            else publish_operand<OpT, C, MI, NJ, STRIDE, true>(base, acc, rowmask);
+        }
     };
     prefetch((const OpT*)J.w1[0] + (size_t)ct0 * J.ct1, J.ct1, ctb1);
     __syncthreads();
@@ -207,13 +224,14 @@
             xr[it] = __builtin_bit_cast(f32x4, __builtin_amdgcn_raw_buffer_load_b128(rs_src, v0[it / 8] + (unsigned)((it % 8) * (C * 4)), 0, 0));
         }
     };
+    constexpr int NTH = NTL / 2;
     const unsigned dl_lds = lds_address(T) + (unsigned)(lrow * TSTR + (ct0 * 32 + half4) * 4);
     using lds_f32x4 = __attribute__((address_space(3))) f32x4;
     if constexpr (KL == 2) issue_loads(r0);
 
     auto do_step = [&](auto fillc, const int step) {
         constexpr bool FILL = decltype(fillc)::value;
-        f32x16 xin[MI][NJ];
+        acc_t xin[MIH][NTL];
         if constexpr (KL == 2) {
             bar();
             if constexpr (xhf) {
@@ -231,12 +249,12 @@
                     unsigned b0 = dlh_lds;
                     asm volatile("" : "+v"(b0));
 #pragma unroll
-                    for (int jt = 0; jt < NJ; ++jt)
-#pragma unroll
-                        for (int mi = 0; mi < MI; ++mi)
-#pragma unroll
-                            for (int g = 0; g < 4; ++g) {
-                                const h4 v = *(const lds_h4*)(size_t)(b0 + (unsigned)(jt * 32 * TSTRH + (mi * 32 + 8 * g) * 2));
+                    for (int jt = 0; jt < NTL; ++jt)
+#pragma unroll
+                        for (int mi = 0; mi < MIH; ++mi)
+#pragma unroll
+                            for (int g = 0; g < NG; ++g) {
+                                const h4 v = *(const lds_h4*)(size_t)(b0 + (unsigned)(jt * TR * TSTRH + (mi * CT + 8 * g) * 2));
 #pragma unroll
                                 for (int e = 0; e < 4; ++e) xin[mi][jt][4 * g + e] = (float)v[e];
                             }
@@ -250,15 +268,15 @@
             }
             bar();
             {
-                unsigned b0 = dl_lds, b1 = dl_lds + (unsigned)(3 * 32 * TSTR);
+                unsigned b0 = dl_lds, b1 = dl_lds + (unsigned)(NTH * TR * TSTR);
                 asm volatile("" : "+v"(b0), "+v"(b1));
 #pragma unroll
-                for (int jt = 0; jt < NJ; ++jt)
-#pragma unroll
-                    for (int mi = 0; mi < MI; ++mi)
-#pragma unroll
-                        for (int g = 0; g < 4; ++g) {
-                            const f32x4 v = *(const lds_f32x4*)(size_t)((jt < 3 ? b0 : b1) + (unsigned)((jt % 3) * 32 * TSTR + (mi * 32 + 8 * g) * 4));
+                for (int jt = 0; jt < NTL; ++jt)
+#pragma unroll
+                    for (int mi = 0; mi < MIH; ++mi)
+#pragma unroll
+                        for (int g = 0; g < NG; ++g) {
+                            const f32x4 v = *(const lds_f32x4*)(size_t)((jt < NTH ? b0 : b1) + (unsigned)((jt % NTH) * TR * TSTR + (mi * CT + 8 * g) * 4));
 #pragma unroll
                             for (int e = 0; e < 4; ++e) xin[mi][jt][4 * g + e] = v[e];
                         }
@@ -286,7 +304,7 @@
         stamp(8);
         auto pair = [&](auto mc) {
             constexpr int m = decltype(mc)::value;
-            using jt0_t = std::integral_constant<int, FILL ? rs_fill_inst(m, NJ) : 0>;
+            using jt0_t = std::integral_constant<int, FILL ? LAG * rs_fill_inst(m, NJ) : 0>;
             const int dil = J.dil[m];
             const int p1 = dil * (J.k - 1) / 2;
             const int Hx = 32 + p1 - p2;
@@ -313,15 +331,14 @@
             }
             rs_copy_rows<STRIDE, NT>(M + (size_t)(RS_HROW - 2 * p2) * STRIDE, sideH, 2 * p2);
             {
-                unsigned rowmask[NJ];
-#pragma unroll
-                for (int jt = 0; jt < NJ; ++jt) {
-                    const int t = wm + jt * 32 + lrow;
+                unsigned rowmask[NTL];
+#pragma unroll
+                for (int jt = 0; jt < NTL; ++jt) {
+                    const int t = wm + jt * TR + lrow;
                     rowmask[jt] = (t >= 0 && t < L) ? 0xffffffffu : 0u;
                 }
                 char* xw = M + (size_t)(RS_HEAD + lrow) * STRIDE + (ct0 * 32 + half4) * 2;
-                if (interior) publish_operand<OpT, C, MI, NJ, STRIDE, false>(xw, xin, rowmask);
-                else publish_operand<OpT, C, MI, NJ, STRIDE, true>(xw, xin, rowmask);
+                publish(xw, xin, rowmask, interior);
                 if constexpr (KL == 2) {
 #pragma unroll
                     for (int it = 0; it < NIT; ++it) {
@@ -329,48 +346,50 @@
                         *(uint4*)(M + (size_t)(RS_HEAD - Hx + i) * STRIDE + ct0 * 64 + (lane % WCH) * 16) = hb[it];
                     }
 #pragma unroll
-                    for (int jt = NJ - 2; jt < NJ; ++jt) {
-                        const int srow = jt * 32 + lrow - (R - Hx);
+                    for (int jt = NTL - 2 * LAG; jt < NTL; ++jt) {
+                        const int srow = jt * TR + lrow - (R - Hx);
                         char* tw = (srow >= 0 ? sideX + (size_t)srow * STRIDE : dump) + (ct0 * 32 + half4) * 2;
 #pragma unroll
-                        for (int mi = 0; mi < MI; ++mi)
-#pragma unroll
-                            for (int g = 0; g < 4; ++g) {
-                                const f32x16& t = xin[mi][jt];
-                                *(uint2*)(tw + (mi * 32 + 8 * g) * 2) =
+                        for (int mi = 0; mi < MIH; ++mi)
+#pragma unroll
+                            for (int g = 0; g < NG; ++g) {
+                                const acc_t& t = xin[mi][jt];
+                                *(uint2*)(tw + (mi * CT + 8 * g) * 2) =
                                     interior ? pack4_lrelu<OpT, false>(t[4 * g + 0], t[4 * g + 1], t[4 * g + 2], t[4 * g + 3], 0u)
                                              : pack4_lrelu<OpT, true>(t[4 * g + 0], t[4 * g + 1], t[4 * g + 2], t[4 * g + 3], rowmask[jt]);
                             }
                     }
                 }
             }
-            f32x16 res[MI][NJ];
-#pragma unroll
-            for (int mi = 0; mi < MI; ++mi) {
-                res[mi][0] = carry[m][mi];
-#pragma unroll
-                for (int jt = 1; jt < NJ; ++jt) res[mi][jt] = xin[mi][jt - 1];
-                carry[m][mi] = xin[mi][NJ - 1];
+            acc_t res[MIH][NTL];
+#pragma unroll
+            for (int mi = 0; mi < MIH; ++mi) {
+#pragma unroll
+                for (int jt = 0; jt < LAG; ++jt) res[mi][jt] = carry[m][mi][jt];
+#pragma unroll
+                for (int jt = LAG; jt < NTL; ++jt) res[mi][jt] = xin[mi][jt - LAG];
+#pragma unroll
+                for (int jt = 0; jt < LAG; ++jt) carry[m][mi][jt] = xin[mi][NTL - LAG + jt];
             }
             stamp(0);
             bar();
             stamp(1);
 
-            f32x16 hacc[MI][NJ];
+            acc_t hacc[MIH][NTL];
             {
                 const float* bl = bias_l + (m * 2 + 0) * CP + ct0 * 32 + half4;
 #pragma unroll
-                for (int mi = 0; mi < MI; ++mi)
-#pragma unroll
-                    for (int g = 0; g < 4; ++g) {
-                        const f32x4 bv = *(const f32x4*)(bl + mi * 32 + 8 * g);
-#pragma unroll
-                        for (int jt = 0; jt < NJ; ++jt)
+                for (int mi = 0; mi < MIH; ++mi)
+#pragma unroll
+                    for (int g = 0; g < NG; ++g) {
+                        const f32x4 bv = *(const f32x4*)(bl + mi * CT + 8 * g);
+#pragma unroll
+                        for (int jt = 0; jt < NTL; ++jt)
 #pragma unroll
                             for (int e = 0; e < 4; ++e) hacc[mi][jt][4 * g + e] = bv[e];
                     }
             }
-            run(jt0_t{}, hacc, M + (size_t)(RS_HEAD - Hx + lrow) * STRIDE + (lane >> 5) * 16, w1l, J.ct1, ctb1, dil);
+            run(jt0_t{}, hacc, M + (size_t)(RS_HEAD - Hx + lrow) * STRIDE + bchunk(), w1l, J.ct1, ctb1, dil);
             prefetch(w2l, J.ct2, ctb2);
             stamp(2);
             bar();
@@ -379,25 +398,27 @@
             if constexpr (KL != 2) rs_copy_rows<STRIDE, NT>(sideX, M + (size_t)(RS_HEAD + R - Hx) * STRIDE, Hx);
             {
                 const int am = wm - 32 + p2;
-                unsigned rowmask[NJ];
-#pragma unroll
-                for (int jt = 0; jt < NJ; ++jt) {
-                    const int t = am + jt * 32 + lrow;
+                unsigned rowmask[NTL];
+#pragma unroll
+                for (int jt = 0; jt < NTL; ++jt) {
+                    const int t = am + jt * TR + lrow;
                     rowmask[jt] = (t >= 0 && t < L) ? 0xffffffffu : 0u;
                 }
                 char* hw = M + (size_t)(RS_HROW + lrow) * STRIDE + (ct0 * 32 + half4) * 2;
-                if (interior) publish_operand<OpT, C, MI, NJ, STRIDE, false>(hw, hacc, rowmask);
-                else publish_operand<OpT, C, MI, NJ, STRIDE, true>(hw, hacc, rowmask);
-                const int srow = lrow - (32 - 2 * p2);
-                char* tw = (srow >= 0 ? sideH + (size_t)srow * STRIDE : dump) + (ct0 * 32 + half4) * 2;
-#pragma unroll
-                for (int mi = 0; mi < MI; ++mi)
-#pragma unroll
-                    for (int g = 0; g < 4; ++g) {
-                        const f32x16& t = hacc[mi][NJ - 1];
-                        *(uint2*)(tw + (mi * 32 + 8 * g) * 2) =
-                            pack4_lrelu<OpT, true>(t[4 * g + 0], t[4 * g + 1], t[4 * g + 2], t[4 * g + 3], rowmask[NJ - 1]);
-                    }
+                publish(hw, hacc, rowmask, interior);
+#pragma unroll
+                for (int jt = NTL - LAG; jt < NTL; ++jt) {
+                    const int srow = jt * TR + lrow - (R - 2 * p2);
+                    char* tw = (srow >= 0 ? sideH + (size_t)srow * STRIDE : dump) + (ct0 * 32 + half4) * 2;
+#pragma unroll
+                    for (int mi = 0; mi < MIH; ++mi)
+#pragma unroll
+                        for (int g = 0; g < NG; ++g) {
+                            const acc_t& t = hacc[mi][jt];
+                            *(uint2*)(tw + (mi * CT + 8 * g) * 2) =
+                                pack4_lrelu<OpT, true>(t[4 * g + 0], t[4 * g + 1], t[4 * g + 2], t[4 * g + 3], rowmask[jt]);
+                        }
+                }
             }
             stamp(4);
             bar();
@@ -406,17 +427,17 @@
             {
                 const float* bl = bias_l + (m * 2 + 1) * CP + ct0 * 32 + half4;
 #pragma unroll
-                for (int mi = 0; mi < MI; ++mi)
-#pragma unroll
-                    for (int g = 0; g < 4; ++g) {
-                        const f32x4 bv = *(const f32x4*)(bl + mi * 32 + 8 * g);
-#pragma unroll
-                        for (int jt = 0; jt < NJ; ++jt)
+                for (int mi = 0; mi < MIH; ++mi)
+#pragma unroll
+                    for (int g = 0; g < NG; ++g) {
+                        const f32x4 bv = *(const f32x4*)(bl + mi * CT + 8 * g);
+#pragma unroll
+                        for (int jt = 0; jt < NTL; ++jt)
 #pragma unroll
                             for (int e = 0; e < 4; ++e) res[mi][jt][4 * g + e] += bv[e];
                     }
             }
-            run(jt0_t{}, res, M + (size_t)(RS_HROW - 2 * p2 + lrow) * STRIDE + (lane >> 5) * 16, w2l, J.ct2, ctb2, 1);
+            run(jt0_t{}, res, M + (size_t)(RS_HROW - 2 * p2 + lrow) * STRIDE + bchunk(), w2l, J.ct2, ctb2, 1);
             {
                 const int mn = (m + 1 < ND) ? m + 1 : 0;
                 prefetch((const OpT*)J.w1[mn] + (size_t)ct0 * J.ct1, J.ct1, ctb1);
@@ -425,9 +446,9 @@
             bar();
             stamp(7);
 #pragma unroll
-            for (int mi = 0; mi < MI; ++mi)
-#pragma unroll
-                for (int jt = 0; jt < NJ; ++jt) xin[mi][jt] = res[mi][jt];
+            for (int mi = 0; mi < MIH; ++mi)
+#pragma unroll
+                for (int jt = 0; jt < NTL; ++jt) xin[mi][jt] = res[mi][jt];
         };
         pair(std::integral_constant<int, 0>{});
         if constexpr (ND > 1) pair(std::integral_constant<int, 1>{});
@@ -444,12 +465,12 @@
                     unsigned b0 = dlh_lds;
                     asm volatile("" : "+v"(b0));
 #pragma unroll
-                    for (int jt = 0; jt < NJ; ++jt)
-#pragma unroll
-                        for (int mi = 0; mi < MI; ++mi)
-#pragma unroll
-                            for (int g = 0; g < 4; ++g)
-                                *(lds_u2*)(size_t)(b0 + (unsigned)(jt * 32 * TSTRH + (mi * 32 + 8 * g) * 2)) = __builtin_bit_cast(
+                    for (int jt = 0; jt < NTL; ++jt)
+#pragma unroll
+                        for (int mi = 0; mi < MIH; ++mi)
+#pragma unroll
+                            for (int g = 0; g < NG; ++g)
+                                *(lds_u2*)(size_t)(b0 + (unsigned)(jt * TR * TSTRH + (mi * CT + 8 * g) * 2)) = __builtin_bit_cast(
                                     u32x2_t, pack4_h(xin[mi][jt][4 * g + 0], xin[mi][jt][4 * g + 1], xin[mi][jt][4 * g + 2], xin[mi][jt][4 * g + 3]));
                 }
                 bar();
@@ -465,16 +486,16 @@
                 }
             } else {
             {
-                unsigned b0 = dl_lds, b1 = dl_lds + (unsigned)(3 * 32 * TSTR);
+                unsigned b0 = dl_lds, b1 = dl_lds + (unsigned)(NTH * TR * TSTR);
                 asm volatile("" : "+v"(b0), "+v"(b1));
 #pragma unroll
-                for (int jt = 0; jt < NJ; ++jt)
-#pragma unroll
-                    for (int mi = 0; mi < MI; ++mi)
-#pragma unroll
-                        for (int g = 0; g < 4; ++g) {
+                for (int jt = 0; jt < NTL; ++jt)
+#pragma unroll
+                    for (int mi = 0; mi < MIH; ++mi)
+#pragma unroll
+                        for (int g = 0; g < NG; ++g) {
                             const f32x4 v = {xin[mi][jt][4 * g + 0], xin[mi][jt][4 * g + 1], xin[mi][jt][4 * g + 2], xin[mi][jt][4 * g + 3]};
-                            *(lds_f32x4*)(size_t)((jt < 3 ? b0 : b1) + (unsigned)((jt % 3) * 32 * TSTR + (mi * 32 + 8 * g) * 4)) = v;
+                            *(lds_f32x4*)(size_t)((jt < NTH ? b0 : b1) + (unsigned)((jt % NTH) * TR * TSTR + (mi * CT + 8 * g) * 4)) = v;
                         }
             }
             bar();
```

Measured after the change: 5905 x real-time (audio-sec/wall-sec), whole job (median of 6 runs). 2.5% higher.
